# CyberAgentAILab/layout-dm

Measured on NVIDIA H100. Metric: layouts_per_sec_T100_batch1024_N25, higher is better.
Workload: dtype fp16

## Files before the change

layoutdm_b200/csrc/common.cuh:

```cuda
#pragma once
#include <cuda.h>
#include <cuda_bf16.h>
#include <cuda_fp16.h>
#include <cuda_runtime.h>
#include <stdint.h>

namespace ldm {

#define LDM_DEVINL __device__ __forceinline__

constexpr float kLogEps = -69.07755278982137f;

LDM_DEVINL uint32_t smem_u32(const void* p) { return static_cast<uint32_t>(__cvta_generic_to_shared(p)); }
LDM_DEVINL void st_shared_u32(uint32_t addr, uint32_t v) { asm volatile("st.shared.u32 [%0], %1;" ::"r"(addr), "r"(v) : "memory"); }

LDM_DEVINL void pdl_wait() { asm volatile("griddepcontrol.wait;" ::: "memory"); }
LDM_DEVINL void pdl_launch_dependents() { asm volatile("griddepcontrol.launch_dependents;" ::: "memory"); }
LDM_DEVINL void pdl_sync() { pdl_wait(); pdl_launch_dependents(); }

LDM_DEVINL void mbar_init(uint64_t* bar, uint32_t count) {
  asm volatile("mbarrier.init.shared::cta.b64 [%0], %1;" ::"r"(smem_u32(bar)), "r"(count) : "memory");
}
LDM_DEVINL void fence_mbar_init() { asm volatile("fence.mbarrier_init.release.cluster;" ::: "memory"); }

LDM_DEVINL void mbar_arrive_expect_tx(uint64_t* bar, uint32_t bytes) {
  asm volatile("mbarrier.arrive.expect_tx.shared::cta.b64 _, [%0], %1;" ::"r"(smem_u32(bar)), "r"(bytes) : "memory");
}
LDM_DEVINL void mbar_arrive(uint64_t* bar) {
  asm volatile("mbarrier.arrive.shared::cta.b64 _, [%0];" ::"r"(smem_u32(bar)) : "memory");
}
LDM_DEVINL bool mbar_try_wait(uint64_t* bar, uint32_t parity) {
  uint32_t ok;
  asm volatile(
      "{\n\t.reg .pred p;\n\t"
      "mbarrier.try_wait.parity.shared::cta.b64 p, [%1], %2;\n\t"
      "selp.u32 %0, 1, 0, p;\n\t}\n"
      : "=r"(ok)
      : "r"(smem_u32(bar)), "r"(parity)
      : "memory");
  return ok != 0;
}
LDM_DEVINL void mbar_wait(uint64_t* bar, uint32_t parity) {
  uint32_t spins = 0;
  while (!mbar_try_wait(bar, parity)) {
    if (++spins > (1u << 28)) { asm volatile("trap;"); }
  }
}

LDM_DEVINL void tma_prefetch_desc(const CUtensorMap* m) {
  asm volatile("prefetch.tensormap [%0];" ::"l"(reinterpret_cast<uint64_t>(m)) : "memory");
}
LDM_DEVINL void tma_load_2d(void* smem_dst, const CUtensorMap* map, uint64_t* bar, int32_t c0, int32_t c1) {
  asm volatile(
      "cp.async.bulk.tensor.2d.shared::cluster.global.mbarrier::complete_tx::bytes [%0], [%1, {%3, %4}], [%2];"
      ::"r"(smem_u32(smem_dst)), "l"(reinterpret_cast<uint64_t>(map)), "r"(smem_u32(bar)), "r"(c0), "r"(c1)
      : "memory");
}
LDM_DEVINL void tma_store_2d(const CUtensorMap* map, const void* smem_src, int32_t c0, int32_t c1) {
  asm volatile("cp.async.bulk.tensor.2d.global.shared::cta.bulk_group [%0, {%2, %3}], [%1];"
               ::"l"(reinterpret_cast<uint64_t>(map)), "r"(smem_u32(smem_src)), "r"(c0), "r"(c1)
               : "memory");
}
LDM_DEVINL void bulk_copy_g2s(void* smem_dst, const void* src, uint32_t bytes, uint64_t* bar) {
  asm volatile("cp.async.bulk.shared::cluster.global.mbarrier::complete_tx::bytes [%0], [%1], %2, [%3];"
               ::"r"(smem_u32(smem_dst)), "l"(reinterpret_cast<uint64_t>(src)), "r"(bytes), "r"(smem_u32(bar))
               : "memory");
}
LDM_DEVINL void bulk_copy_s2g(void* dst, const void* smem_src, uint32_t bytes) {
  asm volatile("cp.async.bulk.global.shared::cta.bulk_group [%0], [%1], %2;"
               ::"l"(reinterpret_cast<uint64_t>(dst)), "r"(smem_u32(smem_src)), "r"(bytes)
               : "memory");
}
LDM_DEVINL void bulk_commit_group() { asm volatile("cp.async.bulk.commit_group;" ::: "memory"); }
template <int N>
LDM_DEVINL void bulk_wait_group_read() { asm volatile("cp.async.bulk.wait_group.read %0;" ::"n"(N) : "memory"); }
LDM_DEVINL void bulk_wait_group_all() { asm volatile("cp.async.bulk.wait_group 0;" ::: "memory"); }
LDM_DEVINL void fence_proxy_async_smem() { asm volatile("fence.proxy.async.shared::cta;" ::: "memory"); }

template <int R>
LDM_DEVINL void setmaxnreg_inc() { asm volatile("setmaxnreg.inc.sync.aligned.u32 %0;" ::"n"(R)); }
template <int R>
LDM_DEVINL void setmaxnreg_dec() { asm volatile("setmaxnreg.dec.sync.aligned.u32 %0;" ::"n"(R)); }

LDM_DEVINL void named_bar_sync(int id, int nthreads) { asm volatile("bar.sync %0, %1;" ::"r"(id), "r"(nthreads) : "memory"); }

LDM_DEVINL void wgmma_fence() { asm volatile("wgmma.fence.sync.aligned;" ::: "memory"); }
LDM_DEVINL void wgmma_commit() { asm volatile("wgmma.commit_group.sync.aligned;" ::: "memory"); }
template <int N>
LDM_DEVINL void wgmma_wait() { asm volatile("wgmma.wait_group.sync.aligned %0;" ::"n"(N) : "memory"); }
template <int N>
LDM_DEVINL void fence_acc(float (&d)[N]) {
#pragma unroll
  for (int i = 0; i < N; ++i) asm volatile("" : "+f"(d[i])::"memory");
}

template <int SW>
LDM_DEVINL uint64_t make_smem_desc(uint32_t smem_addr) {
  static_assert(SW == 128 || SW == 64, "the kernels use the 128- and 64-byte swizzles");
  uint64_t d = 0;
  d |= static_cast<uint64_t>((smem_addr & 0x3FFFF) >> 4);
  d |= static_cast<uint64_t>(1) << 16;
  d |= static_cast<uint64_t>(8 * SW >> 4) << 32;
  d |= static_cast<uint64_t>(SW == 128 ? 1 : 2) << 62;
  return d;
}

#define LDM_F(i) "+f"(d[i])
#define LDM_ACC128 "{%0, %1, %2, %3, %4, %5, %6, %7, %8, %9, %10, %11, %12, %13, %14, %15, %16, %17, %18, %19, %20, %21, %22, %23, %24, %25, %26, %27, %28, %29, %30, %31, %32, %33, %34, %35, %36, %37, %38, %39, %40, %41, %42, %43, %44, %45, %46, %47, %48, %49, %50, %51, %52, %53, %54, %55, %56, %57, %58, %59, %60, %61, %62, %63, %64, %65, %66, %67, %68, %69, %70, %71, %72, %73, %74, %75, %76, %77, %78, %79, %80, %81, %82, %83, %84, %85, %86, %87, %88, %89, %90, %91, %92, %93, %94, %95, %96, %97, %98, %99, %100, %101, %102, %103, %104, %105, %106, %107, %108, %109, %110, %111, %112, %113, %114, %115, %116, %117, %118, %119, %120, %121, %122, %123, %124, %125, %126, %127}"
#define LDM_OUT128 LDM_F(0), LDM_F(1), LDM_F(2), LDM_F(3), LDM_F(4), LDM_F(5), LDM_F(6), LDM_F(7), LDM_F(8), LDM_F(9), LDM_F(10), LDM_F(11), LDM_F(12), LDM_F(13), LDM_F(14), LDM_F(15), LDM_F(16), LDM_F(17), LDM_F(18), LDM_F(19), LDM_F(20), LDM_F(21), LDM_F(22), LDM_F(23), LDM_F(24), LDM_F(25), LDM_F(26), LDM_F(27), LDM_F(28), LDM_F(29), LDM_F(30), LDM_F(31), LDM_F(32), LDM_F(33), LDM_F(34), LDM_F(35), LDM_F(36), LDM_F(37), LDM_F(38), LDM_F(39), LDM_F(40), LDM_F(41), LDM_F(42), LDM_F(43), LDM_F(44), LDM_F(45), LDM_F(46), LDM_F(47), LDM_F(48), LDM_F(49), LDM_F(50), LDM_F(51), LDM_F(52), LDM_F(53), LDM_F(54), LDM_F(55), LDM_F(56), LDM_F(57), LDM_F(58), LDM_F(59), LDM_F(60), LDM_F(61), LDM_F(62), LDM_F(63), LDM_F(64), LDM_F(65), LDM_F(66), LDM_F(67), LDM_F(68), LDM_F(69), LDM_F(70), LDM_F(71), LDM_F(72), LDM_F(73), LDM_F(74), LDM_F(75), LDM_F(76), LDM_F(77), LDM_F(78), LDM_F(79), LDM_F(80), LDM_F(81), LDM_F(82), LDM_F(83), LDM_F(84), LDM_F(85), LDM_F(86), LDM_F(87), LDM_F(88), LDM_F(89), LDM_F(90), LDM_F(91), LDM_F(92), LDM_F(93), LDM_F(94), LDM_F(95), LDM_F(96), LDM_F(97), LDM_F(98), LDM_F(99), LDM_F(100), LDM_F(101), LDM_F(102), LDM_F(103), LDM_F(104), LDM_F(105), LDM_F(106), LDM_F(107), LDM_F(108), LDM_F(109), LDM_F(110), LDM_F(111), LDM_F(112), LDM_F(113), LDM_F(114), LDM_F(115), LDM_F(116), LDM_F(117), LDM_F(118), LDM_F(119), LDM_F(120), LDM_F(121), LDM_F(122), LDM_F(123), LDM_F(124), LDM_F(125), LDM_F(126), LDM_F(127)
#define LDM_ACC116 "{%0, %1, %2, %3, %4, %5, %6, %7, %8, %9, %10, %11, %12, %13, %14, %15, %16, %17, %18, %19, %20, %21, %22, %23, %24, %25, %26, %27, %28, %29, %30, %31, %32, %33, %34, %35, %36, %37, %38, %39, %40, %41, %42, %43, %44, %45, %46, %47, %48, %49, %50, %51, %52, %53, %54, %55, %56, %57, %58, %59, %60, %61, %62, %63, %64, %65, %66, %67, %68, %69, %70, %71, %72, %73, %74, %75, %76, %77, %78, %79, %80, %81, %82, %83, %84, %85, %86, %87, %88, %89, %90, %91, %92, %93, %94, %95, %96, %97, %98, %99, %100, %101, %102, %103, %104, %105, %106, %107, %108, %109, %110, %111, %112, %113, %114, %115}"
#define LDM_OUT116 LDM_F(0), LDM_F(1), LDM_F(2), LDM_F(3), LDM_F(4), LDM_F(5), LDM_F(6), LDM_F(7), LDM_F(8), LDM_F(9), LDM_F(10), LDM_F(11), LDM_F(12), LDM_F(13), LDM_F(14), LDM_F(15), LDM_F(16), LDM_F(17), LDM_F(18), LDM_F(19), LDM_F(20), LDM_F(21), LDM_F(22), LDM_F(23), LDM_F(24), LDM_F(25), LDM_F(26), LDM_F(27), LDM_F(28), LDM_F(29), LDM_F(30), LDM_F(31), LDM_F(32), LDM_F(33), LDM_F(34), LDM_F(35), LDM_F(36), LDM_F(37), LDM_F(38), LDM_F(39), LDM_F(40), LDM_F(41), LDM_F(42), LDM_F(43), LDM_F(44), LDM_F(45), LDM_F(46), LDM_F(47), LDM_F(48), LDM_F(49), LDM_F(50), LDM_F(51), LDM_F(52), LDM_F(53), LDM_F(54), LDM_F(55), LDM_F(56), LDM_F(57), LDM_F(58), LDM_F(59), LDM_F(60), LDM_F(61), LDM_F(62), LDM_F(63), LDM_F(64), LDM_F(65), LDM_F(66), LDM_F(67), LDM_F(68), LDM_F(69), LDM_F(70), LDM_F(71), LDM_F(72), LDM_F(73), LDM_F(74), LDM_F(75), LDM_F(76), LDM_F(77), LDM_F(78), LDM_F(79), LDM_F(80), LDM_F(81), LDM_F(82), LDM_F(83), LDM_F(84), LDM_F(85), LDM_F(86), LDM_F(87), LDM_F(88), LDM_F(89), LDM_F(90), LDM_F(91), LDM_F(92), LDM_F(93), LDM_F(94), LDM_F(95), LDM_F(96), LDM_F(97), LDM_F(98), LDM_F(99), LDM_F(100), LDM_F(101), LDM_F(102), LDM_F(103), LDM_F(104), LDM_F(105), LDM_F(106), LDM_F(107), LDM_F(108), LDM_F(109), LDM_F(110), LDM_F(111), LDM_F(112), LDM_F(113), LDM_F(114), LDM_F(115)
#define LDM_ACC80 "{%0, %1, %2, %3, %4, %5, %6, %7, %8, %9, %10, %11, %12, %13, %14, %15, %16, %17, %18, %19, %20, %21, %22, %23, %24, %25, %26, %27, %28, %29, %30, %31, %32, %33, %34, %35, %36, %37, %38, %39, %40, %41, %42, %43, %44, %45, %46, %47, %48, %49, %50, %51, %52, %53, %54, %55, %56, %57, %58, %59, %60, %61, %62, %63, %64, %65, %66, %67, %68, %69, %70, %71, %72, %73, %74, %75, %76, %77, %78, %79}"
#define LDM_OUT80 LDM_F(0), LDM_F(1), LDM_F(2), LDM_F(3), LDM_F(4), LDM_F(5), LDM_F(6), LDM_F(7), LDM_F(8), LDM_F(9), LDM_F(10), LDM_F(11), LDM_F(12), LDM_F(13), LDM_F(14), LDM_F(15), LDM_F(16), LDM_F(17), LDM_F(18), LDM_F(19), LDM_F(20), LDM_F(21), LDM_F(22), LDM_F(23), LDM_F(24), LDM_F(25), LDM_F(26), LDM_F(27), LDM_F(28), LDM_F(29), LDM_F(30), LDM_F(31), LDM_F(32), LDM_F(33), LDM_F(34), LDM_F(35), LDM_F(36), LDM_F(37), LDM_F(38), LDM_F(39), LDM_F(40), LDM_F(41), LDM_F(42), LDM_F(43), LDM_F(44), LDM_F(45), LDM_F(46), LDM_F(47), LDM_F(48), LDM_F(49), LDM_F(50), LDM_F(51), LDM_F(52), LDM_F(53), LDM_F(54), LDM_F(55), LDM_F(56), LDM_F(57), LDM_F(58), LDM_F(59), LDM_F(60), LDM_F(61), LDM_F(62), LDM_F(63), LDM_F(64), LDM_F(65), LDM_F(66), LDM_F(67), LDM_F(68), LDM_F(69), LDM_F(70), LDM_F(71), LDM_F(72), LDM_F(73), LDM_F(74), LDM_F(75), LDM_F(76), LDM_F(77), LDM_F(78), LDM_F(79)
#define LDM_ACC64 "{%0, %1, %2, %3, %4, %5, %6, %7, %8, %9, %10, %11, %12, %13, %14, %15, %16, %17, %18, %19, %20, %21, %22, %23, %24, %25, %26, %27, %28, %29, %30, %31, %32, %33, %34, %35, %36, %37, %38, %39, %40, %41, %42, %43, %44, %45, %46, %47, %48, %49, %50, %51, %52, %53, %54, %55, %56, %57, %58, %59, %60, %61, %62, %63}"
#define LDM_OUT64 LDM_F(0), LDM_F(1), LDM_F(2), LDM_F(3), LDM_F(4), LDM_F(5), LDM_F(6), LDM_F(7), LDM_F(8), LDM_F(9), LDM_F(10), LDM_F(11), LDM_F(12), LDM_F(13), LDM_F(14), LDM_F(15), LDM_F(16), LDM_F(17), LDM_F(18), LDM_F(19), LDM_F(20), LDM_F(21), LDM_F(22), LDM_F(23), LDM_F(24), LDM_F(25), LDM_F(26), LDM_F(27), LDM_F(28), LDM_F(29), LDM_F(30), LDM_F(31), LDM_F(32), LDM_F(33), LDM_F(34), LDM_F(35), LDM_F(36), LDM_F(37), LDM_F(38), LDM_F(39), LDM_F(40), LDM_F(41), LDM_F(42), LDM_F(43), LDM_F(44), LDM_F(45), LDM_F(46), LDM_F(47), LDM_F(48), LDM_F(49), LDM_F(50), LDM_F(51), LDM_F(52), LDM_F(53), LDM_F(54), LDM_F(55), LDM_F(56), LDM_F(57), LDM_F(58), LDM_F(59), LDM_F(60), LDM_F(61), LDM_F(62), LDM_F(63)
#define LDM_ACC32 "{%0, %1, %2, %3, %4, %5, %6, %7, %8, %9, %10, %11, %12, %13, %14, %15, %16, %17, %18, %19, %20, %21, %22, %23, %24, %25, %26, %27, %28, %29, %30, %31}"
#define LDM_OUT32 LDM_F(0), LDM_F(1), LDM_F(2), LDM_F(3), LDM_F(4), LDM_F(5), LDM_F(6), LDM_F(7), LDM_F(8), LDM_F(9), LDM_F(10), LDM_F(11), LDM_F(12), LDM_F(13), LDM_F(14), LDM_F(15), LDM_F(16), LDM_F(17), LDM_F(18), LDM_F(19), LDM_F(20), LDM_F(21), LDM_F(22), LDM_F(23), LDM_F(24), LDM_F(25), LDM_F(26), LDM_F(27), LDM_F(28), LDM_F(29), LDM_F(30), LDM_F(31)
template <bool BF16>
LDM_DEVINL void wgmma_ss_n256(float (&d)[128], uint64_t da, uint64_t db, uint32_t accumulate) {
  if constexpr (BF16)
    asm volatile("{\n\t.reg .pred p;\n\tsetp.ne.b32 p, %130, 0;\n\t"
                 "wgmma.mma_async.sync.aligned.m64n256k16.f32.bf16.bf16 " LDM_ACC128 ", %128, %129, p, 1, 1, 0, 0;\n\t}\n"
                 : LDM_OUT128 : "l"(da), "l"(db), "r"(accumulate));
  else
    asm volatile("{\n\t.reg .pred p;\n\tsetp.ne.b32 p, %130, 0;\n\t"
                 "wgmma.mma_async.sync.aligned.m64n256k16.f32.f16.f16 " LDM_ACC128 ", %128, %129, p, 1, 1, 0, 0;\n\t}\n"
                 : LDM_OUT128 : "l"(da), "l"(db), "r"(accumulate));
}
template <bool BF16>
LDM_DEVINL void wgmma_ss_n232(float (&d)[116], uint64_t da, uint64_t db, uint32_t accumulate) {
  if constexpr (BF16)
    asm volatile("{\n\t.reg .pred p;\n\tsetp.ne.b32 p, %118, 0;\n\t"
                 "wgmma.mma_async.sync.aligned.m64n232k16.f32.bf16.bf16 " LDM_ACC116 ", %116, %117, p, 1, 1, 0, 0;\n\t}\n"
                 : LDM_OUT116 : "l"(da), "l"(db), "r"(accumulate));
  else
    asm volatile("{\n\t.reg .pred p;\n\tsetp.ne.b32 p, %118, 0;\n\t"
                 "wgmma.mma_async.sync.aligned.m64n232k16.f32.f16.f16 " LDM_ACC116 ", %116, %117, p, 1, 1, 0, 0;\n\t}\n"
                 : LDM_OUT116 : "l"(da), "l"(db), "r"(accumulate));
}
template <bool BF16>
LDM_DEVINL void wgmma_ss_n160(float (&d)[80], uint64_t da, uint64_t db, uint32_t accumulate) {
  if constexpr (BF16)
    asm volatile("{\n\t.reg .pred p;\n\tsetp.ne.b32 p, %82, 0;\n\t"
                 "wgmma.mma_async.sync.aligned.m64n160k16.f32.bf16.bf16 " LDM_ACC80 ", %80, %81, p, 1, 1, 0, 0;\n\t}\n"
                 : LDM_OUT80 : "l"(da), "l"(db), "r"(accumulate));
  else
    asm volatile("{\n\t.reg .pred p;\n\tsetp.ne.b32 p, %82, 0;\n\t"
                 "wgmma.mma_async.sync.aligned.m64n160k16.f32.f16.f16 " LDM_ACC80 ", %80, %81, p, 1, 1, 0, 0;\n\t}\n"
                 : LDM_OUT80 : "l"(da), "l"(db), "r"(accumulate));
}
template <bool BF16>
LDM_DEVINL void wgmma_ss_n128(float (&d)[64], uint64_t da, uint64_t db, uint32_t accumulate) {
  if constexpr (BF16)
    asm volatile("{\n\t.reg .pred p;\n\tsetp.ne.b32 p, %66, 0;\n\t"
                 "wgmma.mma_async.sync.aligned.m64n128k16.f32.bf16.bf16 " LDM_ACC64 ", %64, %65, p, 1, 1, 0, 0;\n\t}\n"
                 : LDM_OUT64 : "l"(da), "l"(db), "r"(accumulate));
  else
    asm volatile("{\n\t.reg .pred p;\n\tsetp.ne.b32 p, %66, 0;\n\t"
                 "wgmma.mma_async.sync.aligned.m64n128k16.f32.f16.f16 " LDM_ACC64 ", %64, %65, p, 1, 1, 0, 0;\n\t}\n"
                 : LDM_OUT64 : "l"(da), "l"(db), "r"(accumulate));
}
template <bool BF16>
LDM_DEVINL void wgmma_rs_n64_tb(float (&d)[32], const uint32_t (&a)[4], uint64_t db, uint32_t accumulate) {
  if constexpr (BF16)
    asm volatile("{\n\t.reg .pred p;\n\tsetp.ne.b32 p, %37, 0;\n\t"
                 "wgmma.mma_async.sync.aligned.m64n64k16.f32.bf16.bf16 " LDM_ACC32 ", {%32, %33, %34, %35}, %36, p, 1, 1, 1;\n\t}\n"
                 : LDM_OUT32 : "r"(a[0]), "r"(a[1]), "r"(a[2]), "r"(a[3]), "l"(db), "r"(accumulate));
  else
    asm volatile("{\n\t.reg .pred p;\n\tsetp.ne.b32 p, %37, 0;\n\t"
                 "wgmma.mma_async.sync.aligned.m64n64k16.f32.f16.f16 " LDM_ACC32 ", {%32, %33, %34, %35}, %36, p, 1, 1, 1;\n\t}\n"
                 : LDM_OUT32 : "r"(a[0]), "r"(a[1]), "r"(a[2]), "r"(a[3]), "l"(db), "r"(accumulate));
}
#undef LDM_ACC128
#undef LDM_OUT128
#undef LDM_ACC116
#undef LDM_OUT116
#undef LDM_ACC80
#undef LDM_OUT80
#undef LDM_ACC64
#undef LDM_OUT64
#undef LDM_ACC32
#undef LDM_OUT32
#undef LDM_F

enum : int { OP_F16 = 0, OP_BF16 = 1, OP_BF16X3 = 2 };
template <int MODE> struct OpT;
template <> struct OpT<OP_F16> {
  using T = __half; using T2 = __half2;
  static LDM_DEVINL uint32_t pack(float a, float b) { __half2 h = __floats2half2_rn(a, b); return *reinterpret_cast<uint32_t*>(&h); }
  static LDM_DEVINL T from(float a) { return __float2half_rn(a); }
};
template <> struct OpT<OP_BF16> {
  using T = __nv_bfloat16; using T2 = __nv_bfloat162;
  static LDM_DEVINL uint32_t pack(float a, float b) { __nv_bfloat162 h = __floats2bfloat162_rn(a, b); return *reinterpret_cast<uint32_t*>(&h); }
  static LDM_DEVINL T from(float a) { return __float2bfloat16_rn(a); }
};
template <> struct OpT<OP_BF16X3> : OpT<OP_BF16> {
  static LDM_DEVINL void pack_pair(float a, float b, uint32_t& hi, uint32_t& lo) {
    const __nv_bfloat162 h = __floats2bfloat162_rn(a, b);
    const float2 hf = __bfloat1622float2(h);
    const __nv_bfloat162 l = __floats2bfloat162_rn(a - hf.x, b - hf.y);
    hi = *reinterpret_cast<const uint32_t*>(&h); lo = *reinterpret_cast<const uint32_t*>(&l);
  }
  static LDM_DEVINL void from_pair(float a, T& hi, T& lo) { hi = __float2bfloat16_rn(a); lo = __float2bfloat16_rn(a - __bfloat162float(hi)); }
};
template <int MODE> constexpr bool kOpBf16 = MODE != OP_F16;
template <int MODE> constexpr bool kOpSplit = MODE == OP_BF16X3;

template <int MODE> struct OpMaps { CUtensorMap hi; };
template <> struct OpMaps<OP_BF16X3> { CUtensorMap hi, lo; };

LDM_DEVINL uint4 philox4x32_10(uint4 c, uint2 k) {
  constexpr uint32_t M0 = 0xD2511F53u, M1 = 0xCD9E8D57u, W0 = 0x9E3779B9u, W1 = 0xBB67AE85u;
#pragma unroll
  for (int i = 0; i < 10; ++i) {
    const uint32_t hi0 = __umulhi(M0, c.x), lo0 = M0 * c.x;
    const uint32_t hi1 = __umulhi(M1, c.z), lo1 = M1 * c.z;
    c = make_uint4(hi1 ^ c.y ^ k.x, lo1, hi0 ^ c.w ^ k.y, lo0);
    k.x += W0; k.y += W1;
  }
  return c;
}

LDM_DEVINL float u01_from_bits(uint32_t w) { return (static_cast<float>(w >> 9) + 0.5f) * 1.1920928955078125e-07f; }

LDM_DEVINL float gumbel_of(float u) { return -logf(-logf(u + 1e-30f) + 1e-30f); }

LDM_DEVINL uint32_t noise_ctr(uint32_t step, uint32_t stream) { return (step & 0xFFFFFFu) | (stream << 24); }

struct TokenNoise {
  uint2 key; uint32_t tok_lo, tok_hi;
  LDM_DEVINL TokenNoise(unsigned long long seed, unsigned long long b_global0, int b, int S, int s) {
    const unsigned long long tok = (b_global0 + b) * static_cast<unsigned long long>(S) + s;
    key = make_uint2(static_cast<uint32_t>(seed), static_cast<uint32_t>(seed >> 32));
    tok_lo = static_cast<uint32_t>(tok); tok_hi = static_cast<uint32_t>(tok >> 32);
  }
  LDM_DEVINL uint4 block(int blk, uint32_t ctr) const { return philox4x32_10(make_uint4(static_cast<uint32_t>(blk), ctr, tok_lo, tok_hi), key); }
  static LDM_DEVINL int block_of(int c) { return c >> 2; }
  static LDM_DEVINL uint32_t word_of(const uint4& r, int c) { const int k = c & 3; return k == 0 ? r.x : k == 1 ? r.y : k == 2 ? r.z : r.w; }
  LDM_DEVINL void lane_words(int lane, uint32_t ctr, uint32_t (&w)[5]) const {
    const uint4 a = block(block_of(4 * lane), ctr), b = block(block_of(128 + lane), ctr);
    w[0] = word_of(a, 4 * lane); w[1] = word_of(a, 4 * lane + 1); w[2] = word_of(a, 4 * lane + 2); w[3] = word_of(a, 4 * lane + 3);
    w[4] = word_of(b, 128 + lane);
  }
  static constexpr float kGroupMargin = 40.0f;
};

template <int N, class Words>
struct ContractDraw {
  Words words;
  LDM_DEVINL void add_gumbel(const bool (&)[N], float (&lg)[N]) const {
    uint32_t w[N];
    words(1u, w);
#pragma unroll
    for (int j = 0; j < N; ++j) lg[j] += gumbel_of(u01_from_bits(w[j]));
  }
  LDM_DEVINL void exponential(const bool (&)[N], float (&e)[N]) const {
    uint32_t w[N];
    words(0u, w);
#pragma unroll
    for (int j = 0; j < N; ++j) e[j] = -logf(u01_from_bits(w[j]));
  }
};
template <int N, class Words>
LDM_DEVINL ContractDraw<N, Words> contract_draw(Words w) { return ContractDraw<N, Words>{w}; }

struct TorchNoise {
  uint2 key; unsigned long long ctr0; uint32_t tthr;
  __host__ __device__ __forceinline__ TorchNoise(unsigned long long seed, unsigned long long offset, uint32_t tthr_) : ctr0(offset >> 2), tthr(tthr_) {
    key = make_uint2(static_cast<uint32_t>(seed), static_cast<uint32_t>(seed >> 32));
  }
  LDM_DEVINL uint32_t word(uint32_t i) const {
    const uint32_t q = i / tthr, sub = i - q * tthr;
    const unsigned long long ctr = ctr0 + (q >> 2);
    return TokenNoise::word_of(philox4x32_10(make_uint4(static_cast<uint32_t>(ctr), static_cast<uint32_t>(ctr >> 32), sub, 0u), key), q & 3);
  }
  static LDM_DEVINL float uniform(uint32_t w) { return __fmaf_rn(__uint2float_rn(w), 0x1p-32f, 0x1p-33f); }
  static LDM_DEVINL float rand(uint32_t w) { const float u = uniform(w); return u == 1.0f ? 0.0f : u; }
  static LDM_DEVINL float exponential(uint32_t w) { const float u = uniform(w); return u >= 1.0f - 0x1p-24f ? 0x1p-24f : -__logf(u); }
  static constexpr float kGroupMargin = 48.0f;
};

template <int N>
struct TorchDraw {
  TorchNoise exp, gum; uint32_t i_exp, exp_cs, i_gum, S; const int (&cls)[N];
  LDM_DEVINL void add_gumbel(const bool (&on)[N], float (&lg)[N]) const {
#pragma unroll
    for (int j = 0; j < N; ++j) if (on[j]) lg[j] += gumbel_of(TorchNoise::rand(gum.word(i_gum + static_cast<uint32_t>(cls[j]) * S)));
  }
  LDM_DEVINL void exponential(const bool (&on)[N], float (&e)[N]) const {
#pragma unroll
    for (int j = 0; j < N; ++j) e[j] = on[j] ? TorchNoise::exponential(exp.word(i_exp + exp_cs * static_cast<uint32_t>(cls[j]))) : 1.0f;
  }
};

LDM_DEVINL float ex2_approx(float x) {
  float y;
  asm("ex2.approx.ftz.f32 %0, %1;" : "=f"(y) : "f"(x));
  return y;
}

LDM_DEVINL float warp_max(float v) {
#pragma unroll
  for (int o = 16; o > 0; o >>= 1) v = fmaxf(v, __shfl_xor_sync(0xffffffffu, v, o));
  return v;
}
LDM_DEVINL float warp_sum(float v) {
#pragma unroll
  for (int o = 16; o > 0; o >>= 1) v += __shfl_xor_sync(0xffffffffu, v, o);
  return v;
}
LDM_DEVINL double warp_sum_d(double v) {
#pragma unroll
  for (int o = 16; o > 0; o >>= 1) v += __shfl_xor_sync(0xffffffffu, v, o);
  return v;
}

}
```

layoutdm_b200/csrc/gemm_tc.cuh:

```cuda
#pragma once
#include "common.cuh"

namespace ldm {

constexpr int kBM = 128;
constexpr int kWgK = 16;
constexpr int kGemmConsumers = 256;
constexpr int kProducerRegs = 40, kConsumerRegs = 232;

constexpr int gemm_kb(bool split) { return split ? 32 : 64; }

enum : int { EPI_QKV = 0, EPI_RELU = 1, EPI_F32 = 2, EPI_LN = 3 };

struct GemmParams {
  int M, N, K;
  int n_tiles;
  const float* bias;
  void* out;
  int ldo;
  float qscale;
  int qcols;
  const float* resid;
  float* y_out;
  const float* ln_scale;
  const float* ln_shift;
  int adaln;
  float* out32;
  const int* t_layout;
  int n_layouts;
  int rev;
  void* out_lo;
};

template <bool BF16, int N>
LDM_DEVINL void wgmma_ss(float (&d)[N / 2], uint64_t da, uint64_t db, uint32_t accumulate) {
  if constexpr (N == 256) wgmma_ss_n256<BF16>(d, da, db, accumulate);
  else if constexpr (N == 232) wgmma_ss_n232<BF16>(d, da, db, accumulate);
  else if constexpr (N == 160) wgmma_ss_n160<BF16>(d, da, db, accumulate);
  else { static_assert(N == 128, "unsupported wgmma width"); wgmma_ss_n128<BF16>(d, da, db, accumulate); }
}

template <int KB, int PLANES, int A_ROWS, int B_ROWS, int WG_N, int STAGES, bool K_TAIL = true>
struct Ring {
  static constexpr int kKB = KB, kStages = STAGES, kWgN = WG_N;
  static constexpr int kRowBytes = 2 * KB;
  static constexpr int kAPlane = A_ROWS * kRowBytes;
  static constexpr int kABytes = PLANES * kAPlane;
  static constexpr int kBBytes = B_ROWS * kRowBytes;
  static constexpr int kStageBytes = kABytes + PLANES * WG_N * kBBytes;
  static constexpr int kBytes = STAGES * kStageBytes;
  static_assert(kAPlane % (8 * kRowBytes) == 0 && kBBytes % (8 * kRowBytes) == 0, "boxes must keep the swizzle atom's alignment");

  uint8_t* stages;
  uint64_t* full;
  uint64_t* empty;

  LDM_DEVINL Ring(uint8_t* smem, uint64_t* bars) : stages(smem), full(bars), empty(bars + STAGES) {}
  static LDM_DEVINL int num_kb(int K) { return K_TAIL ? (K + KB - 1) / KB : K / KB; }

  template <int MODE>
  static LDM_DEVINL void prefetch(const OpMaps<MODE>& a, const OpMaps<MODE>& b) {
    tma_prefetch_desc(&a.hi);
    tma_prefetch_desc(&b.hi);
    if constexpr (kOpSplit<MODE>) { tma_prefetch_desc(&a.lo); tma_prefetch_desc(&b.lo); }
  }
  LDM_DEVINL void init() const {
    for (int i = 0; i < STAGES; ++i) { mbar_init(&full[i], 1); mbar_init(&empty[i], kGemmConsumers); }
  }
  static LDM_DEVINL void advance(int& s, uint32_t& phase) { if (++s == STAGES) { s = 0; phase ^= 1; } }
  LDM_DEVINL void release_prev(int s) const { mbar_arrive(&empty[s == 0 ? STAGES - 1 : s - 1]); }

  template <int MODE>
  LDM_DEVINL void load_tile(int& s, uint32_t& phase, const OpMaps<MODE>& a, const OpMaps<MODE>& b, int num_kb, int m0, int n0) const {
    static_assert(PLANES == (kOpSplit<MODE> ? 2 : 1), "one operand map per plane");
    for (int kb = 0; kb < num_kb; ++kb) {
      mbar_wait(&empty[s], phase ^ 1);
      uint8_t* st = stages + s * kStageBytes;
      mbar_arrive_expect_tx(&full[s], kStageBytes);
      tma_load_2d(st, &a.hi, &full[s], kb * KB, m0);
#pragma unroll
      for (int wn = 0; wn < WG_N; ++wn) tma_load_2d(st + kABytes + wn * kBBytes, &b.hi, &full[s], kb * KB, n0 + wn * B_ROWS);
      if constexpr (PLANES == 2) {
        tma_load_2d(st + kAPlane, &a.lo, &full[s], kb * KB, m0);
#pragma unroll
        for (int wn = 0; wn < WG_N; ++wn)
          tma_load_2d(st + kABytes + (WG_N + wn) * kBBytes, &b.lo, &full[s], kb * KB, n0 + wn * B_ROWS);
      }
      advance(s, phase);
    }
  }

  template <int MODE>
  LDM_DEVINL void mma_tile(int& s, uint32_t& phase, float (&acc)[B_ROWS / 2], int wm, int wn, int num_kb, int K) const {
    static_assert(PLANES == (kOpSplit<MODE> ? 2 : 1), "one operand map per plane");
    for (int kb = 0; kb < num_kb; ++kb) {
      mbar_wait(&full[s], phase);
      const uint32_t st = smem_u32(stages + s * kStageBytes);
      const uint64_t da = make_smem_desc<kRowBytes>(st + wm * 64 * kRowBytes), da_lo = make_smem_desc<kRowBytes>(st + kAPlane + wm * 64 * kRowBytes);
      const uint64_t db = make_smem_desc<kRowBytes>(st + kABytes + wn * kBBytes);
      const uint64_t db_lo = make_smem_desc<kRowBytes>(st + kABytes + (WG_N + wn) * kBBytes);
      wgmma_fence();
      const auto step = [&](int k) {
        if constexpr (PLANES == 2) {
          wgmma_ss<true, B_ROWS>(acc, da_lo + 2 * k, db + 2 * k, (kb | k) != 0);
          wgmma_ss<true, B_ROWS>(acc, da + 2 * k, db_lo + 2 * k, 1);
          wgmma_ss<true, B_ROWS>(acc, da + 2 * k, db + 2 * k, 1);
        } else {
          wgmma_ss<kOpBf16<MODE>, B_ROWS>(acc, da + 2 * k, db + 2 * k, (kb | k) != 0);
        }
      };
      const bool whole = !K_TAIL || kb * KB + KB <= K;
      if (PLANES == 2 || !whole) step(0);
      if (whole) {
#pragma unroll
        for (int k = PLANES == 2 ? 1 : 0; k < KB / kWgK; ++k) step(k);
      }
      wgmma_commit();
      if (kb > 0) { wgmma_wait<1>(); release_prev(s); }
      advance(s, phase);
    }
    wgmma_wait<0>();
    fence_acc(acc);
    release_prev(s);
  }
};

template <int EPI, bool SPLIT>
constexpr bool kStagedStore = (EPI == EPI_QKV || EPI == EPI_RELU) && !SPLIT;
template <int EPI, int MODE>
constexpr int kGemmThreads = kStagedStore<EPI, kOpSplit<MODE>> ? 384 : 288;

template <int BN_WG, int WG_M, int STAGES, bool SPLIT = false, bool STAGED = false>
struct GemmSmem {
  using R = Ring<gemm_kb(SPLIT), SPLIT ? 2 : 1, 64 * WG_M, BN_WG, 3 - WG_M, STAGES>;
  static constexpr int kStoreCb = 64 * WG_M * 128;
  static constexpr int kStoreBytes = STAGED ? (R::kWgN * BN_WG / 64) * kStoreCb : 0;
  static_assert(!STAGED || BN_WG % 64 == 0, "staged stores go out in 64-column boxes");
  static constexpr int kOffStore = R::kBytes;
  static constexpr int kOffBars = kOffStore + kStoreBytes;
  static constexpr int kOffStat = kOffBars + 256;
  static constexpr int kBytes = kOffStat + 2 * 64 * 16 + 1024 ;
  static_assert(2 * STAGES * 8 <= 256, "barrier block overflow");
  static_assert(kBytes <= 232448, "exceeds the 227 KB of shared memory per CTA");
};

template <int EPI, int N>
LDM_DEVINL void bias_act(const float (&acc)[N], int j, const float* bias, int c, float scale, float (&v)[4]) {
  const float2 b = bias != nullptr ? __ldg(reinterpret_cast<const float2*>(bias + c)) : make_float2(0.0f, 0.0f);
  v[0] = acc[4 * j] + b.x; v[1] = acc[4 * j + 1] + b.y; v[2] = acc[4 * j + 2] + b.x; v[3] = acc[4 * j + 3] + b.y;
#pragma unroll
  for (int e = 0; e < 4; ++e) {
    if constexpr (EPI == EPI_QKV) v[e] *= scale;
    if constexpr (EPI == EPI_RELU) v[e] = fmaxf(v[e], 0.0f);
  }
}

struct LnAffine { const float* gam; const float* bet; float gadd; };
LDM_DEVINL LnAffine ln_affine(const float* scale, const float* shift, int adaln, const int* t_layout, int n_layouts, int m0, int N) {
  LnAffine a{scale, shift, adaln ? 1.0f : 0.0f};
  if (t_layout != nullptr) {
    const int layout = m0 / kBM;
    const int tl = layout < n_layouts ? __ldg(t_layout + layout) : 0;
    a.gam = scale + static_cast<size_t>(tl) * 2 * N; a.bet = a.gam + N; a.gadd = 1.0f;
  }
  return a;
}

template <int BN_WG, int WG_M, int STAGES, int EPI, int MODE>
__global__ void __launch_bounds__(kGemmThreads<EPI, MODE>, 1)
gemm_tc_kernel(const __grid_constant__ OpMaps<MODE> map_a ,
               const __grid_constant__ OpMaps<MODE> map_b ,
               const __grid_constant__ CUtensorMap map_out, const GemmParams p) {
  constexpr bool SPLIT = kOpSplit<MODE>, STAGED = kStagedStore<EPI, SPLIT>;
  using SM = GemmSmem<BN_WG, WG_M, STAGES, SPLIT, STAGED>;
  using O = OpT<MODE>;
  constexpr int kBMt = 64 * WG_M, kAcc = BN_WG / 2;
  static_assert(EPI != EPI_LN || (WG_M == 1 && BN_WG == 232), "LN epilogue is laid out for 464 = 2 x 232 columns");
  static_assert(EPI == EPI_LN || WG_M == 2, "plain epilogues use 128-row tiles");

  extern __shared__ __align__(1024) uint8_t smem_raw[];
  uint8_t* smem = reinterpret_cast<uint8_t*>((reinterpret_cast<uintptr_t>(smem_raw) + 1023) & ~uintptr_t(1023));
  typename SM::R ring(smem, reinterpret_cast<uint64_t*>(smem + SM::kOffBars));

  const int warp = __shfl_sync(0xffffffffu, threadIdx.x >> 5, 0), lane = threadIdx.x & 31;
  const int num_kb = SM::R::num_kb(p.K);
  const int n_mblk = p.M / kBMt, n_work = n_mblk * p.n_tiles;
  const auto tile_m0 = [&](int t) { const int mb = t / p.n_tiles; return (p.rev ? n_mblk - 1 - mb : mb) * kBMt; };
  const auto tile_n0 = [&](int t) { return (t % p.n_tiles) * BN_WG * SM::R::kWgN; };

  if (threadIdx.x == kGemmConsumers) {
    ring.prefetch(map_a, map_b);
    if constexpr (STAGED) tma_prefetch_desc(&map_out);
    ring.init();
    fence_mbar_init();
  }
  __syncthreads();
  pdl_sync();

  if (warp >= kGemmConsumers / 32) {
    if constexpr (STAGED) setmaxnreg_dec<kProducerRegs>();
    if (threadIdx.x == kGemmConsumers) {
      int s = 0;
      uint32_t phase = 0;
      for (int t = blockIdx.x; t < n_work; t += gridDim.x) {
        ring.load_tile(s, phase, map_a, map_b, num_kb, tile_m0(t), tile_n0(t));
        if constexpr (!STAGED) break;
      }
    }
    return;
  }

  if constexpr (STAGED) setmaxnreg_inc<kConsumerRegs>();
  const int wg = warp >> 2;
  const int wm = WG_M == 2 ? wg : 0, wn = WG_M == 2 ? 0 : wg;
  float acc[kAcc];
#pragma unroll
  for (int i = 0; i < kAcc; ++i) acc[i] = 0.0f;
  int s = 0;
  uint32_t phase = 0;
  for (int t = blockIdx.x; t < n_work; t += gridDim.x) {
    const int m0 = tile_m0(t), n0 = tile_n0(t);
    ring.template mma_tile<MODE>(s, phase, acc, wm, wn, num_kb, p.K);

    const int rw = (warp & 3) * 16 + (lane >> 2);
    const int row0 = m0 + wm * 64 + rw, row1 = row0 + 8;
    const int col0 = n0 + wn * BN_WG + 2 * (lane & 3);

    if constexpr (STAGED) {
      float scale = 1.0f;
      if constexpr (EPI == EPI_QKV) scale = (n0 < p.qcols) ? p.qscale : 1.0f;
      const bool leader = (threadIdx.x & 127) == 0;
      uint8_t* stage = smem + SM::kOffStore + wm * 64 * 128;
      const uint32_t stage_u32 = smem_u32(stage);
      const auto wg_bar = [&]() { if (wg == 0) named_bar_sync(2, 128); else named_bar_sync(3, 128); };
      if (leader) bulk_wait_group_read<0>();
      wg_bar();
      const int sw = (rw & 7) << 4;
#pragma unroll
      for (int j = 0; j < BN_WG / 8; ++j) {
        const int c = col0 + 8 * j;
        if (c >= p.N) continue;
        float v[4];
        bias_act<EPI>(acc, j, p.bias, c, scale, v);
        const uint32_t blk = stage_u32 + (j >> 3) * SM::kStoreCb + ((((j & 7) << 4) ^ sw) | (4 * (lane & 3)));
        st_shared_u32(blk + rw * 128, O::pack(v[0], v[1]));
        st_shared_u32(blk + (rw + 8) * 128, O::pack(v[2], v[3]));
      }
      fence_proxy_async_smem();
      wg_bar();
      if (leader) {
#pragma unroll
        for (int cb = 0; cb < BN_WG / 64; ++cb)
          if (n0 + cb * 64 < p.N) tma_store_2d(&map_out, stage + cb * SM::kStoreCb, n0 + cb * 64, m0 + wm * 64);
        bulk_commit_group();
      }
    } else if constexpr (EPI != EPI_LN) {
      float scale = 1.0f;
      if constexpr (EPI == EPI_QKV) scale = (n0 < p.qcols) ? p.qscale : 1.0f;
#pragma unroll
      for (int j = 0; j < BN_WG / 8; ++j) {
        const int c = col0 + 8 * j;
        if (c >= p.N) continue;
        float v[4];
        bias_act<EPI>(acc, j, p.bias, c, scale, v);
        if constexpr (EPI == EPI_F32) {
          float* o = static_cast<float*>(p.out);
          *reinterpret_cast<float2*>(o + static_cast<size_t>(row0) * p.ldo + c) = make_float2(v[0], v[1]);
          *reinterpret_cast<float2*>(o + static_cast<size_t>(row1) * p.ldo + c) = make_float2(v[2], v[3]);
        } else {
          uint32_t* o0 = reinterpret_cast<uint32_t*>(static_cast<typename O::T*>(p.out) + static_cast<size_t>(row0) * p.ldo + c);
          uint32_t* o1 = reinterpret_cast<uint32_t*>(static_cast<typename O::T*>(p.out) + static_cast<size_t>(row1) * p.ldo + c);
          if constexpr (SPLIT) {
            uint32_t* l0 = reinterpret_cast<uint32_t*>(static_cast<typename O::T*>(p.out_lo) + static_cast<size_t>(row0) * p.ldo + c);
            uint32_t* l1 = reinterpret_cast<uint32_t*>(static_cast<typename O::T*>(p.out_lo) + static_cast<size_t>(row1) * p.ldo + c);
            O::pack_pair(v[0], v[1], *o0, *l0);
            O::pack_pair(v[2], v[3], *o1, *l1);
          } else {
            *o0 = O::pack(v[0], v[1]);
            *o1 = O::pack(v[2], v[3]);
          }
        }
      }
    } else {
      float* ssum = reinterpret_cast<float*>(smem + SM::kOffStat);
      float* ssq = ssum + 2 * 64;
      const int N = p.N;
      const float* r0p = p.resid + static_cast<size_t>(row0) * N;
      const float* r1p = p.resid + static_cast<size_t>(row1) * N;
      const float piv0 = __ldg(p.bias) + r0p[0], piv1 = __ldg(p.bias) + r1p[0];
      float s0 = 0.0f, s1 = 0.0f;
#pragma unroll
      for (int j = 0; j < BN_WG / 8; ++j) {
        const int c = col0 + 8 * j;
        const float2 b = __ldg(reinterpret_cast<const float2*>(p.bias + c));
        const float2 ra = *reinterpret_cast<const float2*>(r0p + c), rb = *reinterpret_cast<const float2*>(r1p + c);
        acc[4 * j] += b.x + ra.x; acc[4 * j + 1] += b.y + ra.y;
        acc[4 * j + 2] += b.x + rb.x; acc[4 * j + 3] += b.y + rb.y;
        if (p.y_out != nullptr) {
          *reinterpret_cast<float2*>(p.y_out + static_cast<size_t>(row0) * N + c) = make_float2(acc[4 * j], acc[4 * j + 1]);
          *reinterpret_cast<float2*>(p.y_out + static_cast<size_t>(row1) * N + c) = make_float2(acc[4 * j + 2], acc[4 * j + 3]);
        }
        acc[4 * j] -= piv0; acc[4 * j + 1] -= piv0; acc[4 * j + 2] -= piv1; acc[4 * j + 3] -= piv1;
        s0 += acc[4 * j] + acc[4 * j + 1];
        s1 += acc[4 * j + 2] + acc[4 * j + 3];
      }
#pragma unroll
      for (int o = 1; o <= 2; o <<= 1) {
        s0 += __shfl_xor_sync(0xffffffffu, s0, o);
        s1 += __shfl_xor_sync(0xffffffffu, s1, o);
      }
      if ((lane & 3) == 0) { ssum[wn * 64 + rw] = s0; ssum[wn * 64 + rw + 8] = s1; }
      named_bar_sync(1, kGemmConsumers);
      const float inv_n = 1.0f / static_cast<float>(N);
      const float mean0 = (s0 + ssum[(wn ^ 1) * 64 + rw]) * inv_n, mean1 = (s1 + ssum[(wn ^ 1) * 64 + rw + 8]) * inv_n;
      float q0 = 0.0f, q1 = 0.0f;
#pragma unroll
      for (int j = 0; j < BN_WG / 8; ++j) {
        const float d0 = acc[4 * j] - mean0, d1 = acc[4 * j + 1] - mean0, d2 = acc[4 * j + 2] - mean1, d3 = acc[4 * j + 3] - mean1;
        q0 = fmaf(d0, d0, fmaf(d1, d1, q0));
        q1 = fmaf(d2, d2, fmaf(d3, d3, q1));
      }
#pragma unroll
      for (int o = 1; o <= 2; o <<= 1) {
        q0 += __shfl_xor_sync(0xffffffffu, q0, o);
        q1 += __shfl_xor_sync(0xffffffffu, q1, o);
      }
      if ((lane & 3) == 0) { ssq[wn * 64 + rw] = q0; ssq[wn * 64 + rw + 8] = q1; }
      named_bar_sync(1, kGemmConsumers);
      const float rstd0 = 1.0f / sqrtf(fmaxf((q0 + ssq[(wn ^ 1) * 64 + rw]) * inv_n, 0.0f) + 1e-5f);
      const float rstd1 = 1.0f / sqrtf(fmaxf((q1 + ssq[(wn ^ 1) * 64 + rw + 8]) * inv_n, 0.0f) + 1e-5f);
      const LnAffine a = ln_affine(p.ln_scale, p.ln_shift, p.adaln, p.t_layout, p.n_layouts, m0, N);
      typename O::T* out16 = static_cast<typename O::T*>(p.out);
#pragma unroll
      for (int j = 0; j < BN_WG / 8; ++j) {
        const int c = col0 + 8 * j;
        const float2 g = __ldg(reinterpret_cast<const float2*>(a.gam + c)), h = __ldg(reinterpret_cast<const float2*>(a.bet + c));
        const float v0 = (acc[4 * j] - mean0) * rstd0 * (g.x + a.gadd) + h.x, v1 = (acc[4 * j + 1] - mean0) * rstd0 * (g.y + a.gadd) + h.y;
        const float v2 = (acc[4 * j + 2] - mean1) * rstd1 * (g.x + a.gadd) + h.x, v3 = (acc[4 * j + 3] - mean1) * rstd1 * (g.y + a.gadd) + h.y;
        if constexpr (SPLIT) {
          typename O::T* lo16 = static_cast<typename O::T*>(p.out_lo);
          O::pack_pair(v0, v1, *reinterpret_cast<uint32_t*>(out16 + static_cast<size_t>(row0) * N + c), *reinterpret_cast<uint32_t*>(lo16 + static_cast<size_t>(row0) * N + c));
          O::pack_pair(v2, v3, *reinterpret_cast<uint32_t*>(out16 + static_cast<size_t>(row1) * N + c), *reinterpret_cast<uint32_t*>(lo16 + static_cast<size_t>(row1) * N + c));
        } else {
          *reinterpret_cast<uint32_t*>(out16 + static_cast<size_t>(row0) * N + c) = O::pack(v0, v1);
          *reinterpret_cast<uint32_t*>(out16 + static_cast<size_t>(row1) * N + c) = O::pack(v2, v3);
        }
        if (p.out32 != nullptr) {
          *reinterpret_cast<float2*>(p.out32 + static_cast<size_t>(row0) * N + c) = make_float2(v0, v1);
          *reinterpret_cast<float2*>(p.out32 + static_cast<size_t>(row1) * N + c) = make_float2(v2, v3);
        }
      }
    }
    if constexpr (!STAGED) break;
  }
  if constexpr (STAGED) {
    if ((threadIdx.x & 127) == 0) bulk_wait_group_all();
  }
}

constexpr int kLnThreads = 384, kLnEpiThreads = 96;
struct LnSmem {
  static constexpr int kRows = 64, kWgCols = 232, kCols = 2 * kWgCols;
  using R = Ring<32, 1, kRows, kWgCols, 2, 3, false>;
  static constexpr int kLd = kCols + 8;
  static constexpr int kOffBuf = R::kBytes;
  static constexpr int kOffBars = kOffBuf + kRows * kLd * 4;
  static constexpr int kOffStat = kOffBars + 64;
  static constexpr int kBytes = kOffStat + 3 * kRows * 4 + 1024 ;
  static_assert(kLd * 4 % 16 == 0, "bulk copies need 16-byte aligned rows");
  static_assert(kBytes <= 232448, "exceeds the 227 KB of shared memory per CTA");
};

template <int MODE>
__global__ void __launch_bounds__(kLnThreads, 1)
gemm_ln_kernel(const __grid_constant__ OpMaps<MODE> map_a , const __grid_constant__ OpMaps<MODE> map_b ,
               const GemmParams p) {
  static_assert(!kOpSplit<MODE>, "the split mode runs the fragment-epilogue LN GEMM");
  using SM = LnSmem;
  using O = OpT<MODE>;
  constexpr int kRows = SM::kRows, kWgCols = SM::kWgCols, kLd = SM::kLd, kAcc = kWgCols / 2;
  constexpr int kEpi = kGemmConsumers, kProducer = kEpi + kLnEpiThreads;

  extern __shared__ __align__(1024) uint8_t smem_raw[];
  uint8_t* smem = reinterpret_cast<uint8_t*>((reinterpret_cast<uintptr_t>(smem_raw) + 1023) & ~uintptr_t(1023));
  SM::R ring(smem, reinterpret_cast<uint64_t*>(smem + SM::kOffBars));
  uint64_t* res_full = ring.empty + SM::R::kStages;
  uint64_t* buf_full = res_full + 1;
  float* buf = reinterpret_cast<float*>(smem + SM::kOffBuf);
  float* s_piv = reinterpret_cast<float*>(smem + SM::kOffStat);
  float* s_sum = s_piv + kRows;
  float* s_rstd = s_sum + kRows;

  const int warp = __shfl_sync(0xffffffffu, threadIdx.x >> 5, 0), lane = threadIdx.x & 31;
  const int N = p.N;
  const int num_kb = SM::R::num_kb(p.K);
  const int n_work = p.M / kRows;
  const auto tile_m0 = [&](int t) { return (p.rev ? n_work - 1 - t : t) * kRows; };

  if (threadIdx.x == kProducer) {
    ring.prefetch(map_a, map_b);
    ring.init();
    mbar_init(res_full, 1);
    mbar_init(buf_full, kGemmConsumers);
    fence_mbar_init();
  }
  __syncthreads();
  pdl_sync();

  if (threadIdx.x >= kProducer) {
    if (threadIdx.x == kProducer) {
      uint32_t phase = 0;
      int s = 0;
      for (int t = blockIdx.x; t < n_work; t += gridDim.x) ring.load_tile(s, phase, map_a, map_b, num_kb, tile_m0(t), 0);
    }
    return;
  }

  if (threadIdx.x >= kEpi) {
    const int et = threadIdx.x - kEpi;
    const bool copier = et < 32;
    const uint32_t row_bytes = static_cast<uint32_t>(N) * sizeof(float);
    const float inv_n = 1.0f / static_cast<float>(N);
    constexpr int kVec = kWgCols / 2;
    constexpr int kTotal = kRows * kVec;
    constexpr int kPerThread = (kTotal + kLnEpiThreads - 1) / kLnEpiThreads;
    const auto load_resid = [&](int t) {
      if (lane == 0) mbar_arrive_expect_tx(res_full, kRows * row_bytes);
      __syncwarp();
      const float* src = p.resid + static_cast<size_t>(tile_m0(t)) * N;
      for (int r = lane; r < kRows; r += 32) bulk_copy_g2s(buf + r * kLd, src + static_cast<size_t>(r) * N, row_bytes, res_full);
    };
    const auto store_rows = [&](float* dst) {
      for (int r = lane; r < kRows; r += 32) bulk_copy_s2g(dst + static_cast<size_t>(r) * N, buf + r * kLd, row_bytes);
      bulk_commit_group();
    };
    if (copier) load_resid(blockIdx.x);
    uint32_t bphase = 0;
    for (int t = blockIdx.x; t < n_work; t += gridDim.x) {
      const int m0 = tile_m0(t);
      mbar_wait(buf_full, bphase);
      if (copier && p.y_out != nullptr) store_rows(p.y_out + static_cast<size_t>(m0) * N);
      {
        const int h = (lane >> 2) & 1, q = lane & 3;
#pragma unroll 1
        for (int g = et >> 5; g < kRows / 4; g += kLnEpiThreads / 32) {
          const int r = 4 * g + (lane >> 3);
          const float piv = s_piv[r];
          const float* yr = buf + r * kLd + h * kWgCols + 2 * q;
          float s = 0.0f;
#pragma unroll
          for (int j = 0; j < kWgCols / 8; ++j) {
            const float2 y = *reinterpret_cast<const float2*>(yr + 8 * j);
            s += (y.x - piv) + (y.y - piv);
          }
          s += __shfl_xor_sync(0xffffffffu, s, 1);
          s += __shfl_xor_sync(0xffffffffu, s, 2);
          s += __shfl_xor_sync(0xffffffffu, s, 4);
          float v = 0.0f;
#pragma unroll
          for (int j = 0; j < kWgCols / 8; ++j) {
            const float2 y = *reinterpret_cast<const float2*>(yr + 8 * j);
            const float d0 = fmaf(-s, inv_n, y.x - piv), d1 = fmaf(-s, inv_n, y.y - piv);
            v = fmaf(d0, d0, fmaf(d1, d1, v));
          }
          v += __shfl_xor_sync(0xffffffffu, v, 1);
          v += __shfl_xor_sync(0xffffffffu, v, 2);
          v += __shfl_xor_sync(0xffffffffu, v, 4);
          if ((lane & 7) == 0) { s_sum[r] = s; s_rstd[r] = 1.0f / sqrtf(fmaxf(v * inv_n, 0.0f) + 1e-5f); }
        }
      }
      if (copier) bulk_wait_group_read<0>();
      named_bar_sync(1, kLnEpiThreads);
      const LnAffine a = ln_affine(p.ln_scale, p.ln_shift, p.adaln, p.t_layout, p.n_layouts, m0, N);
      typename O::T* out16 = static_cast<typename O::T*>(p.out);
      const bool keep32 = p.out32 != nullptr;
#pragma unroll 6
      for (int k = 0; k < kPerThread; ++k) {
        const int i = k * kLnEpiThreads + et, r = i / kVec, c = (i - r * kVec) * 4;
        if (i >= kTotal) continue;
        float4* bp = reinterpret_cast<float4*>(buf + r * kLd + c);
        const float4 y = *bp;
        const float4 g = __ldg(reinterpret_cast<const float4*>(a.gam + c)), b = __ldg(reinterpret_cast<const float4*>(a.bet + c));
        const float piv = s_piv[r], s = s_sum[r], rstd = s_rstd[r];
        const float4 v = make_float4(fmaf(fmaf(-s, inv_n, y.x - piv) * rstd, g.x + a.gadd, b.x), fmaf(fmaf(-s, inv_n, y.y - piv) * rstd, g.y + a.gadd, b.y),
                                     fmaf(fmaf(-s, inv_n, y.z - piv) * rstd, g.z + a.gadd, b.z), fmaf(fmaf(-s, inv_n, y.w - piv) * rstd, g.w + a.gadd, b.w));
        *reinterpret_cast<uint2*>(out16 + static_cast<size_t>(m0 + r) * N + c) = make_uint2(O::pack(v.x, v.y), O::pack(v.z, v.w));
        if (keep32) *bp = v;
      }
      if (keep32) fence_proxy_async_smem();
      named_bar_sync(1, kLnEpiThreads);
      if (copier) {
        if (keep32) store_rows(p.out32 + static_cast<size_t>(m0) * N);
        bulk_wait_group_read<0>();
        if (t + static_cast<int>(gridDim.x) < n_work) load_resid(t + gridDim.x);
      }
      bphase ^= 1;
    }
    if (copier) bulk_wait_group_all();
    return;
  }

  const int wn = warp >> 2;
  float acc[kAcc];
  int s = 0;
  uint32_t phase = 0, bphase = 0;
  const int rw = (warp & 3) * 16 + (lane >> 2);
  const int cw = wn * kWgCols + 2 * (lane & 3);
  float* bw = buf + rw * kLd + cw;
  for (int t = blockIdx.x; t < n_work; t += gridDim.x) {
    ring.mma_tile<MODE>(s, phase, acc, 0, wn, num_kb, p.K);
    mbar_wait(res_full, bphase);
    if (cw == 0) { const float b0 = __ldg(p.bias); s_piv[rw] = b0 + bw[0]; s_piv[rw + 8] = b0 + bw[8 * kLd]; }
#pragma unroll
    for (int j = 0; j < kAcc / 4; ++j) {
      const float2 b = __ldg(reinterpret_cast<const float2*>(p.bias + cw + 8 * j));
      float2* y0 = reinterpret_cast<float2*>(bw + 8 * j);
      float2* y1 = reinterpret_cast<float2*>(bw + 8 * kLd + 8 * j);
      const float2 r0 = *y0, r1 = *y1;
      *y0 = make_float2(acc[4 * j] + (b.x + r0.x), acc[4 * j + 1] + (b.y + r0.y));
      *y1 = make_float2(acc[4 * j + 2] + (b.x + r1.x), acc[4 * j + 3] + (b.y + r1.y));
    }
    fence_proxy_async_smem();
    mbar_arrive(buf_full);
    bphase ^= 1;
  }
}

}
```

layoutdm_b200/csrc/ldm_b200.cu:

```cuda
#include <cuda.h>
#include <cuda_runtime.h>

#include <algorithm>
#include <cmath>
#include <cstdarg>
#include <cstdio>
#include <cstdlib>
#include <cstring>
#include <type_traits>
#include <vector>

#include "../../include/ldm_b200.h"
#include "attention.cuh"
#include "common.cuh"
#include "embed.cuh"
#include "gemm_tc.cuh"
#include "posterior_sample.cuh"
#include "relation.cuh"

using namespace ldm;

namespace {

thread_local char g_err[512] = "";
int fail(int code, const char* fmt, ...) {
  va_list ap; va_start(ap, fmt); vsnprintf(g_err, sizeof(g_err), fmt, ap); va_end(ap);
  return code;
}
#define CK(call)                                                                                   \
  do {                                                                                             \
    cudaError_t e__ = (call);                                                                      \
    if (e__ != cudaSuccess) return fail(LDM_ERR_CUDA, "%s failed: %s (%s:%d)", #call, cudaGetErrorString(e__), __FILE__, __LINE__); \
  } while (0)

constexpr int kMaxLayers = 16;
constexpr int kHeadPad = 64;
constexpr int kQkvN = 3 * 8 * kHeadPad;
constexpr int kAttN = 8 * kHeadPad;
constexpr int kMaxLayouts = 32767;
constexpr int kLogitLd = 160;
constexpr int kDModel = 464;
constexpr int kPlainBN = 256;
template <int MODE> constexpr int kPlainStages = kOpSplit<MODE> ? 4 : 3;
constexpr int kHeadBN = 160, kHeadStages = 4;
constexpr int kLnBN = 232, kLnStages = 3;
constexpr int kLnKB = LnSmem::R::kKB;
static_assert(LnSmem::kWgCols == kLnBN && kAttN % kLnKB == 0 && 4 * kDModel % kLnKB == 0 && gemm_kb(true) == kLnKB, "LN GEMM shapes");
template <int MODE> constexpr auto kGemmQkv = gemm_tc_kernel<kPlainBN, 2, kPlainStages<MODE>, EPI_QKV, MODE>;
template <int MODE> constexpr auto kGemmFf1 = gemm_tc_kernel<kPlainBN, 2, kPlainStages<MODE>, EPI_RELU, MODE>;
template <int MODE> constexpr auto kGemmHead = gemm_tc_kernel<kHeadBN, 2, kHeadStages, EPI_F32, MODE>;
template <int MODE> constexpr auto kGemmLn = gemm_tc_kernel<kLnBN, 1, kLnStages, EPI_LN, MODE>;
template <int MODE>
constexpr int kPlainSmem = GemmSmem<kPlainBN, 2, kPlainStages<MODE>, kOpSplit<MODE>, kStagedStore<EPI_QKV, kOpSplit<MODE>>>::kBytes;
constexpr int kHeadSmem = GemmSmem<kHeadBN, 2, kHeadStages>::kBytes;
constexpr int kLnSmem = GemmSmem<kLnBN, 1, kLnStages>::kBytes;
static_assert(GemmSmem<kHeadBN, 2, kHeadStages, true>::kBytes == kHeadSmem && GemmSmem<kLnBN, 1, kLnStages, true>::kBytes == kLnSmem &&
              GemmSmem<kPlainBN, 2, 4, true>::R::kStageBytes == GemmSmem<kPlainBN, 2, 4>::R::kStageBytes,
              "split-mode ring stages must keep the one-plane sizes");
static_assert(kStagedStore<EPI_QKV, false> == kStagedStore<EPI_RELU, false> && kStagedStore<EPI_QKV, true> == kStagedStore<EPI_RELU, true>,
              "QKV and FF1 share one shared-memory size");

using EncodeTiledFn = CUresult (*)(CUtensorMap*, CUtensorMapDataType, cuuint32_t, void*, const cuuint64_t*, const cuuint64_t*,
                                   const cuuint32_t*, const cuuint32_t*, CUtensorMapInterleave, CUtensorMapSwizzle,
                                   CUtensorMapL2promotion, CUtensorMapFloatOOBfill);
EncodeTiledFn g_encode = nullptr;

int load_encode() {
  if (g_encode) return LDM_OK;
  void* fn = nullptr;
  cudaDriverEntryPointQueryResult qres;
  CK(cudaGetDriverEntryPoint("cuTensorMapEncodeTiled", &fn, cudaEnableDefault, &qres));
  if (qres != cudaDriverEntryPointSuccess || fn == nullptr) return fail(LDM_ERR_CUDA, "cuTensorMapEncodeTiled not available");
  g_encode = reinterpret_cast<EncodeTiledFn>(fn);
  return LDM_OK;
}

int make_map(CUtensorMap* m, const void* base, uint64_t rows, uint64_t cols, uint32_t box_rows, int kb, bool bf16) {
  const cuuint64_t dims[2] = {cols, rows};
  const cuuint64_t strides[1] = {cols * 2};
  const cuuint32_t box[2] = {static_cast<cuuint32_t>(kb), box_rows};
  const cuuint32_t estr[2] = {1, 1};
  CUresult r = g_encode(m, bf16 ? CU_TENSOR_MAP_DATA_TYPE_BFLOAT16 : CU_TENSOR_MAP_DATA_TYPE_FLOAT16, 2, const_cast<void*>(base), dims,
                        strides, box, estr, CU_TENSOR_MAP_INTERLEAVE_NONE, kb == 32 ? CU_TENSOR_MAP_SWIZZLE_64B : CU_TENSOR_MAP_SWIZZLE_128B,
                        CU_TENSOR_MAP_L2_PROMOTION_L2_256B, CU_TENSOR_MAP_FLOAT_OOB_FILL_NONE);
  if (r != CUDA_SUCCESS) return fail(LDM_ERR_CUDA, "cuTensorMapEncodeTiled failed (%d) rows=%llu cols=%llu box_rows=%u", (int)r,
                                     (unsigned long long)rows, (unsigned long long)cols, box_rows);
  return LDM_OK;
}

__global__ void logits_scatter_kernel(const float* __restrict__ src, float* __restrict__ dst, int n_layouts, int S, int C) {
  const size_t n = static_cast<size_t>(n_layouts) * S * C;
  for (size_t i = blockIdx.x * static_cast<size_t>(blockDim.x) + threadIdx.x; i < n; i += static_cast<size_t>(gridDim.x) * blockDim.x) {
    const int c = static_cast<int>(i % C); const size_t tok = i / C; const int s = static_cast<int>(tok % S); const size_t b = tok / S;
    dst[(b * 128 + s) * kLogitLd + c] = src[i];
  }
}
__global__ void logits_gather_kernel(const float* __restrict__ src, float* __restrict__ dst, int n_layouts, int S, int C) {
  const size_t n = static_cast<size_t>(n_layouts) * S * C;
  for (size_t i = blockIdx.x * static_cast<size_t>(blockDim.x) + threadIdx.x; i < n; i += static_cast<size_t>(gridDim.x) * blockDim.x) {
    const int c = static_cast<int>(i % C); const size_t tok = i / C; const int s = static_cast<int>(tok % S); const size_t b = tok / S;
    dst[i] = src[(b * 128 + s) * kLogitLd + c];
  }
}
__global__ void fill_ids_kernel(long long* dst, long long v, size_t n) {
  for (size_t i = blockIdx.x * static_cast<size_t>(blockDim.x) + threadIdx.x; i < n; i += static_cast<size_t>(gridDim.x) * blockDim.x) dst[i] = v;
}

}

struct LdmHandle {
  LdmModelDesc desc;
  int C = 0, S = 0, L = 0, T = 0, G = 0;
  int mode = OP_F16;
  bool bf16 = false;
  bool split = false;
  int64_t launches = 0;
  int pdl = 1;
  int debug_stop_after = 0;
  bool prof = false;
  struct ProfRec { int cat; cudaEvent_t a, b; };
  std::vector<ProfRec> prof_recs;
  float *cat_emb = nullptr, *pos = nullptr, *adaln = nullptr, *sched = nullptr, *lae = nullptr;
  void *wqkv[kMaxLayers] = {}, *wo[kMaxLayers] = {}, *w1[kMaxLayers] = {}, *w2[kMaxLayers] = {}, *whead = nullptr;
  float *bqkv[kMaxLayers] = {}, *bo[kMaxLayers] = {}, *b1[kMaxLayers] = {}, *b2[kMaxLayers] = {}, *ln2w[kMaxLayers] = {}, *ln2b[kMaxLayers] = {};
  float *hlnw = nullptr, *hlnb = nullptr;
  CUtensorMap m_wqkv[kMaxLayers], m_wo[kMaxLayers], m_w1[kMaxLayers], m_w2[kMaxLayers], m_whead;
  void *wqkv_lo[kMaxLayers] = {}, *wo_lo[kMaxLayers] = {}, *w1_lo[kMaxLayers] = {}, *w2_lo[kMaxLayers] = {}, *whead_lo = nullptr;
  CUtensorMap m_wqkv_lo[kMaxLayers], m_wo_lo[kMaxLayers], m_w1_lo[kMaxLayers], m_w2_lo[kMaxLayers], m_whead_lo;
  int *qmap = nullptr, *amap = nullptr, *hmap = nullptr;
  int cap = 0;
  void *x16 = nullptr, *qkv16 = nullptr, *att16 = nullptr, *z16 = nullptr, *hid16 = nullptr;
  float *x32 = nullptr, *y32 = nullptr, *logits = nullptr;
  float* rel_lp = nullptr;
  long long* ids[2] = {nullptr, nullptr};
  long long* ids_final = nullptr;
  long long *c_seq = nullptr, *c_seq_orig = nullptr; unsigned char* c_mask = nullptr; float* c_tbl = nullptr;
  CUtensorMap m_x16, m_z16, m_qkv16;
  CUtensorMap m_att16, m_hid16;
  CUtensorMap m_qkv16_st, m_hid16_st;
  void *x16_lo = nullptr, *qkv16_lo = nullptr, *att16_lo = nullptr, *z16_lo = nullptr, *hid16_lo = nullptr;
  CUtensorMap m_x16_lo, m_z16_lo, m_qkv16_lo, m_att16_lo, m_hid16_lo;
  std::vector<void*> owned;
  int use_graph = 1;
  int sweep = 1;
  int num_sms = 0;
  int max_threads_sm = 0;
  int gemm_ctas = 0;
  int fuse_embed = 1;
  cudaStream_t cap_stream = nullptr;
  cudaGraphExec_t graph_exec = nullptr;
  uint64_t graph_key = 0;
  unsigned long long* call_block = nullptr;
  uint64_t ws_generation = 0;
  int64_t graph_launches = 0;
  std::vector<void*> staging;
};

namespace {

template <typename T>
int dev_alloc(LdmHandle* h, T** p, size_t n) {
  CK(cudaMalloc(reinterpret_cast<void**>(p), n * sizeof(T)));
  h->owned.push_back(*p);
  return LDM_OK;
}
template <typename T>
int dev_upload(LdmHandle* h, T** p, const T* src, size_t n) {
  int rc = dev_alloc(h, p, n);
  if (rc) return rc;
  CK(cudaMemcpy(*p, src, n * sizeof(T), cudaMemcpyHostToDevice));
  return LDM_OK;
}

template <typename T>
int dev_upload_tmp(LdmHandle* h, T** p, const T* src, size_t n) {
  CK(cudaMalloc(reinterpret_cast<void**>(p), n * sizeof(T)));
  h->staging.push_back(*p);
  CK(cudaMemcpy(*p, src, n * sizeof(T), cudaMemcpyHostToDevice));
  return LDM_OK;
}
void free_staging(LdmHandle* h) {
  for (void* p : h->staging) cudaFree(p);
  h->staging.clear();
}

int alloc16(LdmHandle* h, void** dst, void** dst_lo, int rows, int cols) {
  const size_t bytes = static_cast<size_t>(rows) * cols * 2;
  CK(cudaMalloc(dst, bytes));
  h->owned.push_back(*dst);
  if (h->split) { CK(cudaMalloc(dst_lo, bytes)); h->owned.push_back(*dst_lo); }
  return LDM_OK;
}

int pack16(const LdmHandle* h, void* dst, void* dst_lo, const float* src_dev, const int* row_map_dev, int dst_rows, int dst_cols, int src_cols,
           cudaStream_t st, const int* col_map_dev = nullptr) {
  const int blocks = 512;
  if (h->mode == OP_BF16X3) pack_weight_kernel<OP_BF16X3><<<blocks, 256, 0, st>>>(src_dev, dst, row_map_dev, col_map_dev, dst_rows, dst_cols, src_cols, dst_lo);
  else if (h->mode == OP_BF16) pack_weight_kernel<OP_BF16><<<blocks, 256, 0, st>>>(src_dev, dst, row_map_dev, col_map_dev, dst_rows, dst_cols, src_cols, nullptr);
  else pack_weight_kernel<OP_F16><<<blocks, 256, 0, st>>>(src_dev, dst, row_map_dev, col_map_dev, dst_rows, dst_cols, src_cols, nullptr);
  CK(cudaGetLastError());
  return LDM_OK;
}

struct WeightField { const float* LdmWeights::*member; const char* name; size_t n; };
std::vector<WeightField> weight_fields(const LdmHandle* h) {
  const size_t d = h->desc.d_model, ff = h->desc.d_ff, L = h->L, T = h->T, C = h->C, S = h->S;
  return {{&LdmWeights::cat_emb, "cat_emb", C * d},         {&LdmWeights::pos_table, "pos_table", S * d},
          {&LdmWeights::in_proj_w, "in_proj_w", L * 3 * d * d}, {&LdmWeights::in_proj_b, "in_proj_b", L * 3 * d},
          {&LdmWeights::out_proj_w, "out_proj_w", L * d * d},   {&LdmWeights::out_proj_b, "out_proj_b", L * d},
          {&LdmWeights::linear1_w, "linear1_w", L * ff * d},    {&LdmWeights::linear1_b, "linear1_b", L * ff},
          {&LdmWeights::linear2_w, "linear2_w", L * d * ff},    {&LdmWeights::linear2_b, "linear2_b", L * d},
          {&LdmWeights::norm1_emb, "norm1_emb", L * T * d},     {&LdmWeights::norm1_w, "norm1_w", L * 2 * d * d},
          {&LdmWeights::norm1_b, "norm1_b", L * 2 * d},         {&LdmWeights::norm2_w, "norm2_w", L * d},
          {&LdmWeights::norm2_b, "norm2_b", L * d},             {&LdmWeights::head_ln_w, "head_ln_w", d},
          {&LdmWeights::head_ln_b, "head_ln_b", d},             {&LdmWeights::head_w, "head_w", C * d}};
}

int pack_weights(LdmHandle* h, const LdmWeights& w, cudaStream_t st) {
  const int d = h->desc.d_model, ff = h->desc.d_ff, L = h->L, T = h->T;
  const auto copy = [&](float* dst, const float* src, size_t n) { return cudaMemcpyAsync(dst, src, n * sizeof(float), cudaMemcpyDeviceToDevice, st); };
  CK(copy(h->cat_emb, w.cat_emb, static_cast<size_t>(h->C) * d));
  CK(copy(h->pos, w.pos_table, static_cast<size_t>(h->S) * d));
  CK(copy(h->hlnw, w.head_ln_w, d));
  CK(copy(h->hlnb, w.head_ln_b, d));
  adaln_table_kernel<<<dim3(T, L), 256, d * sizeof(float), st>>>(w.norm1_emb, w.norm1_w, w.norm1_b, h->adaln, T, d);
  CK(cudaGetLastError());
  int rc;
  for (int l = 0; l < L; ++l) {
    const size_t dd = static_cast<size_t>(d) * d;
    if ((rc = pack16(h, h->wqkv[l], h->wqkv_lo[l], w.in_proj_w + l * 3 * dd, h->qmap, kQkvN, d, d, st))) return rc;
    qkv_bias_kernel<<<(kQkvN + 255) / 256, 256, 0, st>>>(w.in_proj_b + static_cast<size_t>(l) * 3 * d, h->qmap, h->bqkv[l], kQkvN,
                                                        2 * 8 * kHeadPad, kHeadPad, d / h->desc.n_heads);
    CK(cudaGetLastError());
    if ((rc = pack16(h, h->wo[l], h->wo_lo[l], w.out_proj_w + l * dd, nullptr, d, kAttN, d, st, h->amap))) return rc;
    CK(copy(h->bo[l], w.out_proj_b + static_cast<size_t>(l) * d, d));
    if ((rc = pack16(h, h->w1[l], h->w1_lo[l], w.linear1_w + l * ff * static_cast<size_t>(d), nullptr, ff, d, d, st))) return rc;
    CK(copy(h->b1[l], w.linear1_b + static_cast<size_t>(l) * ff, ff));
    if ((rc = pack16(h, h->w2[l], h->w2_lo[l], w.linear2_w + l * ff * static_cast<size_t>(d), nullptr, d, ff, ff, st))) return rc;
    CK(copy(h->b2[l], w.linear2_b + static_cast<size_t>(l) * d, d));
    CK(copy(h->ln2w[l], w.norm2_w + static_cast<size_t>(l) * d, d));
    CK(copy(h->ln2b[l], w.norm2_b + static_cast<size_t>(l) * d, d));
  }
  return pack16(h, h->whead, h->whead_lo, w.head_w, h->hmap, kLogitLd, d, d, st);
}

int make_op_maps(const LdmHandle* h, CUtensorMap* m, CUtensorMap* m_lo, const void* base, const void* base_lo, uint64_t rows, uint64_t cols,
                 uint32_t box_rows, int kb) {
  int rc = make_map(m, base, rows, cols, box_rows, kb, h->bf16);
  if (rc || !h->split) return rc;
  return make_map(m_lo, base_lo, rows, cols, box_rows, kb, h->bf16);
}

template <int MODE>
OpMaps<MODE> op_maps(const CUtensorMap& hi, const CUtensorMap& lo) {
  OpMaps<MODE> m;
  m.hi = hi;
  if constexpr (kOpSplit<MODE>) m.lo = lo;
  else (void)lo;
  return m;
}

void build_schedule(const LdmModelDesc& d, int N, float* out ) {
  const int T = d.num_timesteps, TT = T + 1;
  std::vector<double> att(T + 1), ctt(T + 1);
  att[0] = 1.0; ctt[0] = 0.0;
  for (int i = 0; i < T; ++i) {
    att[i + 1] = static_cast<double>(i) / (T - 1) * (d.att_T - d.att_1) + d.att_1;
    ctt[i + 1] = static_cast<double>(i) / (T - 1) * (d.ctt_T - d.ctt_1) + d.ctt_1;
  }
  auto l1m = [](double la) { return std::log(1.0 - std::exp(la) + 1e-40); };
  for (int i = 0; i < TT; ++i) for (int r = 0; r < 8; ++r) out[r * TT + i] = 0.0f;
  for (int i = 0; i < T; ++i) {
    const double at = att[i + 1] / att[i];
    const double ct = 1.0 - (1.0 - ctt[i + 1]) / (1.0 - ctt[i]);
    const double bt = (1.0 - at - ct) / N;
    out[0 * TT + i] = static_cast<float>(std::log(at));
    out[1 * TT + i] = static_cast<float>(std::log(bt));
    out[2 * TT + i] = static_cast<float>(std::log(ct));
    out[6 * TT + i] = static_cast<float>(l1m(std::log(ct)));
  }
  for (int i = 0; i < TT; ++i) {
    const double a = (i < T) ? att[i + 1] : 1.0, c = (i < T) ? ctt[i + 1] : 0.0;
    const double b = (1.0 - a - c) / N;
    out[3 * TT + i] = static_cast<float>(std::log(a));
    out[4 * TT + i] = static_cast<float>(std::log(b));
    out[5 * TT + i] = static_cast<float>(std::log(c));
    out[7 * TT + i] = static_cast<float>(l1m(std::log(c)));
  }
}

enum : int { CAT_EMBED = 0, CAT_QKV, CAT_ATTN, CAT_OUTPROJ, CAT_FF1, CAT_FF2, CAT_HEAD, CAT_EPILOGUE, CAT_MISC, CAT_COUNT };

struct ProfScope {
  LdmHandle* h; cudaStream_t st; cudaEvent_t b = nullptr;
  ProfScope(LdmHandle* h_, int cat, cudaStream_t st_) : h(h_), st(st_) {
    h->launches++;
    if (h->prof) {
      cudaEvent_t a; cudaEventCreate(&a); cudaEventCreate(&b);
      cudaEventRecord(a, st);
      h->prof_recs.push_back({cat, a, b});
    }
  }
  ~ProfScope() { if (b) cudaEventRecord(b, st); }
};

template <typename... KArgs, typename... Args>
cudaError_t launch_step(const LdmHandle* h, void (*kernel)(KArgs...), dim3 grid, int block, int smem, cudaStream_t st, Args&&... args) {
  cudaLaunchConfig_t cfg = {};
  cfg.gridDim = grid; cfg.blockDim = dim3(block); cfg.dynamicSmemBytes = smem; cfg.stream = st;
  cudaLaunchAttribute at[1];
  cfg.attrs = at; cfg.numAttrs = 0;
  if (h->pdl) { at[0].id = cudaLaunchAttributeProgrammaticStreamSerialization; at[0].val.programmaticStreamSerializationAllowed = 1; cfg.numAttrs = 1; }
  return cudaLaunchKernelEx(&cfg, kernel, std::forward<Args>(args)...);
}

template <int MODE>
int set_smem() {
  constexpr auto attr = cudaFuncAttributeMaxDynamicSharedMemorySize;
  CK(cudaFuncSetAttribute(kGemmQkv<MODE>, attr, kPlainSmem<MODE>));
  CK(cudaFuncSetAttribute(kGemmFf1<MODE>, attr, kPlainSmem<MODE>));
  CK(cudaFuncSetAttribute(kGemmHead<MODE>, attr, kHeadSmem));
  if constexpr (kOpSplit<MODE>) CK(cudaFuncSetAttribute(kGemmLn<MODE>, attr, kLnSmem));
  else CK(cudaFuncSetAttribute(gemm_ln_kernel<MODE>, attr, LnSmem::kBytes));
  CK(cudaFuncSetAttribute(attention_kernel<MODE>, attr, kOpSplit<MODE> ? kAttSmemBytesSplit : kAttSmemBytes));
  return LDM_OK;
}

void free_workspace(LdmHandle* h) {
  void** ws[] = {&h->x16, &h->qkv16, &h->att16, &h->z16, &h->hid16, &h->x16_lo, &h->qkv16_lo, &h->att16_lo, &h->z16_lo, &h->hid16_lo,
                 reinterpret_cast<void**>(&h->x32), reinterpret_cast<void**>(&h->y32),
                 reinterpret_cast<void**>(&h->logits), reinterpret_cast<void**>(&h->ids[0]), reinterpret_cast<void**>(&h->ids[1]),
                 reinterpret_cast<void**>(&h->ids_final), reinterpret_cast<void**>(&h->c_seq), reinterpret_cast<void**>(&h->c_seq_orig),
                 reinterpret_cast<void**>(&h->c_mask), reinterpret_cast<void**>(&h->rel_lp)};
  for (void** p : ws) { if (*p) cudaFree(*p); *p = nullptr; }
  h->cap = 0;
}

int ensure_workspace(LdmHandle* h, int n_layouts) {
  if (n_layouts > kMaxLayouts) return fail(LDM_ERR_UNSUPPORTED, "batch of %d layouts exceeds the %d a call supports", n_layouts, kMaxLayouts);
  if (n_layouts <= h->cap) return LDM_OK;
  CK(cudaDeviceSynchronize());
  free_workspace(h);
  const size_t M = static_cast<size_t>(n_layouts) * kBM;
  const int d = h->desc.d_model, ff = h->desc.d_ff;
  if (h->split) {
    void** lo[] = {&h->x16_lo, &h->qkv16_lo, &h->att16_lo, &h->z16_lo, &h->hid16_lo};
    const size_t cols[] = {static_cast<size_t>(d), static_cast<size_t>(kQkvN), static_cast<size_t>(kAttN), static_cast<size_t>(d), static_cast<size_t>(ff)};
    for (int i = 0; i < 5; ++i) {
      const cudaError_t e = cudaMalloc(lo[i], M * cols[i] * 2);
      if (e != cudaSuccess) {
        cudaGetLastError();
        free_workspace(h);
        return fail(LDM_ERR_CUDA, "split-operand workspace for %d layouts does not fit: %s", n_layouts, cudaGetErrorString(e));
      }
      CK(cudaMemset(*lo[i], 0, M * cols[i] * 2));
    }
  }
  CK(cudaMalloc(&h->x16, M * d * 2));
  CK(cudaMalloc(&h->qkv16, M * kQkvN * 2));
  CK(cudaMalloc(&h->att16, M * kAttN * 2));
  CK(cudaMalloc(&h->z16, M * d * 2));
  CK(cudaMalloc(&h->hid16, M * ff * 2));
  CK(cudaMalloc(reinterpret_cast<void**>(&h->x32), M * d * 4));
  CK(cudaMalloc(reinterpret_cast<void**>(&h->y32), M * d * 4));
  CK(cudaMalloc(reinterpret_cast<void**>(&h->logits), M * kLogitLd * 4));
  const size_t nid = static_cast<size_t>(n_layouts) * h->S;
  CK(cudaMalloc(reinterpret_cast<void**>(&h->ids[0]), nid * 8));
  CK(cudaMalloc(reinterpret_cast<void**>(&h->ids[1]), nid * 8));
  CK(cudaMalloc(reinterpret_cast<void**>(&h->ids_final), nid * 8));
  CK(cudaMalloc(reinterpret_cast<void**>(&h->c_seq), nid * 8));
  CK(cudaMalloc(reinterpret_cast<void**>(&h->c_seq_orig), nid * 8));
  CK(cudaMalloc(reinterpret_cast<void**>(&h->c_mask), nid));
  CK(cudaMemset(h->x16, 0, M * d * 2)); CK(cudaMemset(h->qkv16, 0, M * kQkvN * 2)); CK(cudaMemset(h->att16, 0, M * kAttN * 2));
  CK(cudaMemset(h->z16, 0, M * d * 2)); CK(cudaMemset(h->hid16, 0, M * ff * 2)); CK(cudaMemset(h->x32, 0, M * d * 4));
  CK(cudaMemset(h->y32, 0, M * d * 4));
  CK(cudaMemset(h->logits, 0, M * kLogitLd * 4));
  h->cap = n_layouts;
  h->ws_generation++;
  int rc;
  const int kb = gemm_kb(h->split);
  if ((rc = make_op_maps(h, &h->m_x16, &h->m_x16_lo, h->x16, h->x16_lo, M, d, kBM, kb))) return rc;
  if ((rc = make_op_maps(h, &h->m_z16, &h->m_z16_lo, h->z16, h->z16_lo, M, d, kBM, kb))) return rc;
  if ((rc = make_op_maps(h, &h->m_att16, &h->m_att16_lo, h->att16, h->att16_lo, M, kAttN, 64, kLnKB))) return rc;
  if ((rc = make_op_maps(h, &h->m_hid16, &h->m_hid16_lo, h->hid16, h->hid16_lo, M, ff, 64, kLnKB))) return rc;
  if ((rc = make_op_maps(h, &h->m_qkv16, &h->m_qkv16_lo, h->qkv16, h->qkv16_lo, M, kQkvN, kBM, kHeadPad))) return rc;
  if (!h->split && (rc = make_map(&h->m_qkv16_st, h->qkv16, M, kQkvN, 64, 64, h->bf16))) return rc;
  if (!h->split && (rc = make_map(&h->m_hid16_st, h->hid16, M, ff, 64, 64, h->bf16))) return rc;
  return LDM_OK;
}

template <int MODE>
int launch_denoiser(LdmHandle* h, int n, const long long* ids_in, int t_model, cudaStream_t st, const int* t_layout = nullptr, bool skip_embed = false) {
  const auto maps = [](const CUtensorMap& hi, const CUtensorMap& lo) { return op_maps<MODE>(hi, lo); };
  const int d = h->desc.d_model, ff = h->desc.d_ff, L = h->L, T = h->T;
  const int M = n * kBM;
  const auto grid = [&](int tiles, bool persistent) {
    if (!persistent) return dim3(tiles);
    return dim3(std::min({tiles, h->num_sms, h->gemm_ctas > 0 ? h->gemm_ctas : tiles}));
  };
  const CUtensorMap no_store{};
  constexpr bool kStaged = kStagedStore<EPI_QKV, kOpSplit<MODE>>;
  const auto ln_gemm = [&](const OpMaps<MODE>& a, const OpMaps<MODE>& w, const GemmParams& p) {
    if constexpr (kOpSplit<MODE>) return launch_step(h, kGemmLn<MODE>, grid(M / 64, false), kGemmThreads<EPI_LN, MODE>, kLnSmem, st, a, w, no_store, p);
    else return launch_step(h, gemm_ln_kernel<MODE>, grid(M / 64, true), kLnThreads, LnSmem::kBytes, st, a, w, p);
  };
  int done = 0;
  int dir = 0;
  auto next_rev = [&]() { dir ^= 1; return h->sweep ? dir : 0; };
#define LDM_STAGE_DONE() do { if (h->debug_stop_after && ++done >= h->debug_stop_after) { CK(cudaGetLastError()); return LDM_OK; } } while (0)
  if (!skip_embed) {
    const int warps = n * 128, blocks = (warps * 32 + 255) / 256;
    ProfScope ps(h, CAT_EMBED, st);
    CK(launch_step(h, embed_adaln_kernel<MODE>, dim3(blocks), 256, 0, st, ids_in, (const float*)h->cat_emb, (const float*)h->pos,
                   (const float*)h->adaln, t_model, t_layout, h->x32, h->x16, n, n, h->S, d, h->x16_lo));
  }
  if (!skip_embed) LDM_STAGE_DONE();
  for (int l = 0; l < L; ++l) {
    {
      GemmParams p{M, kQkvN, d, kQkvN / kPlainBN, h->bqkv[l], h->qkv16, kQkvN, 1.0f / sqrtf(static_cast<float>(d / h->desc.n_heads)), 8 * kHeadPad};
      p.rev = next_rev(); p.out_lo = h->qkv16_lo;
      ProfScope ps(h, CAT_QKV, st);
      CK(launch_step(h, kGemmQkv<MODE>, grid(p.n_tiles * n, kStaged), kGemmThreads<EPI_QKV, MODE>, kPlainSmem<MODE>, st, maps(h->m_x16, h->m_x16_lo), maps(h->m_wqkv[l], h->m_wqkv_lo[l]),
                     kStaged ? h->m_qkv16_st : no_store, p));
    }
    LDM_STAGE_DONE();
    {
      ProfScope ps(h, CAT_ATTN, st);
      CK(launch_step(h, attention_kernel<MODE>, dim3(n * h->desc.n_heads), kAttThreads, kOpSplit<MODE> ? kAttSmemBytesSplit : kAttSmemBytes, st,
                     maps(h->m_qkv16, h->m_qkv16_lo), h->att16, h->S, h->desc.n_heads, n, next_rev(), h->att16_lo));
    }
    LDM_STAGE_DONE();
    {
      GemmParams p{M, d, kAttN, 1, h->bo[l], h->z16, d, 1.0f, 0, h->x32, h->y32, h->ln2w[l], h->ln2b[l], 0, nullptr};
      p.rev = next_rev(); p.out_lo = h->z16_lo;
      ProfScope ps(h, CAT_OUTPROJ, st);
      CK(ln_gemm(maps(h->m_att16, h->m_att16_lo), maps(h->m_wo[l], h->m_wo_lo[l]), p));
    }
    LDM_STAGE_DONE();
    {
      GemmParams p{M, ff, d, (ff + kPlainBN - 1) / kPlainBN, h->b1[l], h->hid16, ff, 1.0f, 0};
      p.rev = next_rev(); p.out_lo = h->hid16_lo;
      ProfScope ps(h, CAT_FF1, st);
      CK(launch_step(h, kGemmFf1<MODE>, grid(p.n_tiles * n, kStaged), kGemmThreads<EPI_RELU, MODE>, kPlainSmem<MODE>, st, maps(h->m_z16, h->m_z16_lo), maps(h->m_w1[l], h->m_w1_lo[l]),
                     kStaged ? h->m_hid16_st : no_store, p));
    }
    LDM_STAGE_DONE();
    {
      GemmParams p{M, d, ff, 1, h->b2[l], nullptr, d, 1.0f, 0, h->y32, nullptr, nullptr, nullptr, 0, nullptr};
      if (l + 1 < L) {
        const float* tab = h->adaln + (static_cast<size_t>(l + 1) * T + t_model) * 2 * d;
        p.ln_scale = tab; p.ln_shift = tab + d; p.adaln = 1; p.out32 = h->x32; p.out = h->x16; p.out_lo = h->x16_lo;
        if (t_layout) { p.ln_scale = h->adaln + static_cast<size_t>(l + 1) * T * 2 * d; p.t_layout = t_layout; p.n_layouts = n; }
      } else {
        p.ln_scale = h->hlnw; p.ln_shift = h->hlnb; p.adaln = 0; p.out32 = nullptr; p.out = h->z16; p.out_lo = h->z16_lo;
      }
      p.rev = next_rev();
      ProfScope ps(h, CAT_FF2, st);
      CK(ln_gemm(maps(h->m_hid16, h->m_hid16_lo), maps(h->m_w2[l], h->m_w2_lo[l]), p));
    }
    LDM_STAGE_DONE();
  }
  {
    GemmParams p{M, kLogitLd, d, 1, nullptr, h->logits, kLogitLd, 1.0f, 0};
    p.rev = next_rev();
    ProfScope ps(h, CAT_HEAD, st);
    CK(launch_step(h, kGemmHead<MODE>, grid(n, false), kGemmThreads<EPI_F32, MODE>, kHeadSmem, st, maps(h->m_z16, h->m_z16_lo), maps(h->m_whead, h->m_whead_lo), no_store, p));
  }
#undef LDM_STAGE_DONE
  CK(cudaGetLastError());
  return LDM_OK;
}

int run_denoiser(LdmHandle* h, int n, const long long* ids_in, int t_model, cudaStream_t st, const int* t_layout = nullptr, bool skip_embed = false) {
  switch (h->mode) {
    case OP_BF16X3: return launch_denoiser<OP_BF16X3>(h, n, ids_in, t_model, st, t_layout, skip_embed);
    case OP_BF16: return launch_denoiser<OP_BF16>(h, n, ids_in, t_model, st, t_layout, skip_embed);
    default: return launch_denoiser<OP_F16>(h, n, ids_in, t_model, st, t_layout, skip_embed);
  }
}

int validate_common(LdmHandle* h, int B, const LdmSampling* s) {
  if (!h) return fail(LDM_ERR_INVALID, "null handle");
  if (B <= 0) return fail(LDM_ERR_INVALID, "batch size must be positive (got %d)", B);
  if (!s) return fail(LDM_ERR_INVALID, "null sampling config");
  if (s->mode < 0 || s->mode > LDM_SAMPLING_GUMBEL) return fail(LDM_ERR_INVALID, "unknown sampling mode %d (sampling.py:118 raises NotImplementedError)", s->mode);
  if (s->mode != LDM_SAMPLING_DETERMINISTIC && !(s->temperature > 0.0f)) return fail(LDM_ERR_INVALID, "temperature must be > 0");
  if (s->mode == LDM_SAMPLING_TOP_P && !(s->top_p > 0.0f && s->top_p <= 1.0f)) return fail(LDM_ERR_INVALID, "top_p must be in (0, 1] (sampling.py:96)");
  if (s->mode == LDM_SAMPLING_TOP_K && !(s->top_k >= 1 && s->top_k <= h->C)) return fail(LDM_ERR_INVALID, "top_k out of range");
  return LDM_OK;
}

struct TorchPolicy { uint32_t tthr, delta; };
TorchPolicy torch_policy(const LdmHandle* h, int64_t numel) {
  const int64_t grid = std::min<int64_t>(static_cast<int64_t>(h->num_sms) * (h->max_threads_sm / 256), (numel + 255) / 256);
  const int64_t tthr = 256 * grid;
  return {static_cast<uint32_t>(tthr), static_cast<uint32_t>(((numel - 1) / (tthr * 4) + 1) * 4)};
}
int64_t torch_numel(const LdmHandle* h, int64_t total_layouts) { return total_layouts * h->S * h->C; }
bool torch_batch_fits(const LdmHandle* h, int64_t total_layouts) {
  return total_layouts <= ((int64_t(1) << 31) - 1) / (static_cast<int64_t>(h->S) * h->C);
}

int validate_noise(const LdmHandle* h, int B, int64_t b_global0, const LdmNoise* nz) {
  if (!nz) return fail(LDM_ERR_INVALID, "null noise description");
  if (nz->kind != LDM_NOISE_CONTRACT && nz->kind != LDM_NOISE_TORCH) return fail(LDM_ERR_INVALID, "unknown noise kind %d", nz->kind);
  if (nz->kind == LDM_NOISE_TORCH) {
    if (b_global0 < 0 || nz->total_layouts < b_global0 + B)
      return fail(LDM_ERR_INVALID, "total_layouts=%lld must cover layouts [%lld, %lld)", (long long)nz->total_layouts, (long long)b_global0, (long long)(b_global0 + B));
    if (!torch_batch_fits(h, nz->total_layouts))
      return fail(LDM_ERR_UNSUPPORTED, "torch-generator noise needs total_layouts * S * C < 2^31 (torch splits larger draws)");
    if (nz->offset % 4) return fail(LDM_ERR_INVALID, "a torch generator offset is a multiple of 4 (got %llu)", (unsigned long long)nz->offset);
  }
  return LDM_OK;
}

StepParams base_step_params(const LdmHandle* h, int B) {
  StepParams p{};
  p.n_layouts = B; p.S = h->S; p.C = h->C; p.n_attr = h->desc.n_attr;
  p.pad_id = h->C - 2; p.mask_id = h->C - 1;
  p.constrained = h->desc.q_type == 0;
  for (int g = 0; g < h->desc.n_attr && g < kMaxAttr; ++g) {
    p.grp_start[g] = g == 0 ? 0 : h->desc.n_cat + (g - 1) * h->desc.n_bins;
    p.grp_n[g] = g == 0 ? h->desc.n_cat : h->desc.n_bins;
  }
  p.T = h->T; p.sched = h->sched; p.lae = h->lae;
  p.logits = h->logits; p.ld_logits = kLogitLd;
  p.mode = SAMP_DETERMINISTIC; p.temperature = 1.0f;
  return p;
}

int step_impl(LdmHandle* h, int B, const long long* ids_in, int t_model, int t_post, const LdmCond* cond, const LdmSampling* samp,
              const LdmNoise& noise, uint32_t step_ctr, int t_step, int64_t b_global0, long long* ids_out, float* logits_out, float* logprob_out,
              const float* logits_in, const float* logprob_in, cudaStream_t st, const unsigned long long* call = nullptr,
              bool skip_embed = false, int t_next = -1) {
  if (t_model < 0 || t_model >= h->T || t_post < 0 || t_post >= h->T)
    return fail(LDM_ERR_INVALID, "timestep out of range: t_model=%d t_post=%d T=%d (constrained.py:139)", t_model, t_post, h->T);
  int rc = ensure_workspace(h, B);
  if (rc) return rc;
  if (logprob_in == nullptr) {
    if (logits_in != nullptr) {
      ProfScope ps(h, CAT_MISC, st);
      logits_scatter_kernel<<<1024, 256, 0, st>>>(logits_in, h->logits, B, h->S, h->C);
    } else {
      rc = run_denoiser(h, B, ids_in, t_model, st, nullptr, skip_embed);
      if (rc) return rc;
    }
    if (logits_out != nullptr) {
      ProfScope ps(h, CAT_MISC, st);
      logits_gather_kernel<<<1024, 256, 0, st>>>(h->logits, logits_out, B, h->S, h->C);
    }
  }
  StepParams p = base_step_params(h, B);
  p.t_post = t_post; p.logprob_in = logprob_in; p.ids_in = ids_in;
  if (cond && cond->seq) {
    p.cond_seq = reinterpret_cast<const long long*>(cond->seq); p.cond_mask = cond->mask;
    p.cond_seq_orig = reinterpret_cast<const long long*>(cond->seq_orig); p.refine_tbl = cond->refine_table;
    p.cond_flags = (cond->mask ? COND_HAS_MASK : 0) | (cond->pad_disable ? COND_PAD_DISABLE : 0) |
                   ((cond->seq_orig && cond->refine_table) ? COND_REFINE : 0);
  }
  p.mode = samp->mode; p.temperature = samp->temperature; p.top_p = samp->top_p; p.top_k = samp->top_k;
  p.seed = noise.seed; p.step_ctr = step_ctr; p.b_global0 = b_global0; p.call = call;
  const bool torch_noise = noise.kind == LDM_NOISE_TORCH;
  if (torch_noise) {
    const TorchPolicy tp = torch_policy(h, torch_numel(h, noise.total_layouts));
    p.t_offset = noise.offset; p.t_tthr = tp.tthr; p.t_delta = tp.delta; p.t_step = t_step; p.t_total = noise.total_layouts;
  }
  const auto generic = torch_noise ? posterior_sample_kernel<TorchNoise> : posterior_sample_kernel<TokenNoise>;
  const auto group = torch_noise ? posterior_sample_group_kernel<TorchNoise> : posterior_sample_group_kernel<TokenNoise>;
  p.ids_out = ids_out; p.logprob_out = logprob_out;
  if (t_next >= 0) {
    p.emb_cat = h->cat_emb; p.emb_pos = h->pos; p.emb_adaln = h->adaln + static_cast<size_t>(t_next) * 2 * h->desc.d_model;
    p.emb_x32 = h->x32; p.emb_x16 = h->x16; p.emb_d = h->desc.d_model; p.emb_bf16 = h->bf16 ? 1 : 0;
  }
  const int warps = B * h->S, blocks = (warps * 32 + 255) / 256;
  const bool relation = cond && cond->seq && cond->rel_adj && logprob_in == nullptr && cond->rel_num_update > 0 && t_model >= 10;
  if (relation) {
    if (h->desc.n_attr != 5 || h->desc.n_elem + 1 > kRelMaxNodes || h->desc.n_bins > 32)
      return fail(LDM_ERR_UNSUPPORTED, "relation update needs the c-x-y-w-h layout with <= 31 elements and <= 32 bins");
    if (!h->rel_lp) CK(cudaMalloc(reinterpret_cast<void**>(&h->rel_lp), static_cast<size_t>(h->cap) * h->S * h->C * sizeof(float)));
    StepParams p1 = p;
    p1.cond_flags &= ~COND_PAD_DISABLE; p1.logprob_out = h->rel_lp; p1.emb_adaln = nullptr;
    {
      ProfScope ps(h, CAT_EPILOGUE, st);
      CK(launch_step(h, generic, blocks, 256, 0, st, p1));
    }
    RelationParams r{};
    r.n_layouts = B; r.S = h->S; r.C = h->C; r.n_attr = h->desc.n_attr; r.n_elem = h->desc.n_elem; r.n_cat = h->desc.n_cat;
    r.n_bins = h->desc.n_bins; r.pad_id = h->C - 2; r.lp = h->rel_lp; r.cond_seq = p.cond_seq; r.adj = cond->rel_adj; r.centers = cond->rel_centers;
    const int btot = cond->rel_batch_total > 0 ? cond->rel_batch_total : B;
    r.step = cond->rel_lambda / static_cast<float>(btot * 14);
    r.n_update = cond->rel_num_update;
    {
      ProfScope ps(h, CAT_EPILOGUE, st);
      CK(launch_step(h, relation_update_kernel, B, kRelThreads, 0, st, r));
    }
    StepParams p2 = p;
    p2.logprob_in = h->rel_lp;
    p2.logprob_out = logprob_out;
    {
      ProfScope ps(h, CAT_EPILOGUE, st);
      CK(launch_step(h, generic, blocks, 256, 0, st, p2));
    }
    CK(cudaGetLastError());
    return LDM_OK;
  }
  {
    ProfScope ps(h, CAT_EPILOGUE, st);
    if (group_kernel_applies(p)) CK(launch_step(h, group, blocks, 256, 0, st, p));
    else CK(launch_step(h, generic, blocks, 256, 0, st, p));
  }
  CK(cudaGetLastError());
  return LDM_OK;
}

}

extern "C" {

const char* ldm_last_error(void) { return g_err; }
const char* ldm_version(void) { return "ldm_b200 0.2 (sm_90a, wgmma)"; }

int ldm_create(const LdmModelDesc* desc, const LdmWeights* w, LdmHandle** out) {
  if (!desc || !w || !out) return fail(LDM_ERR_INVALID, "null argument");
  const int d = desc->d_model, ff = desc->d_ff, L = desc->n_layers, T = desc->num_timesteps;
  const int C = desc->n_cat + 4 * desc->n_bins + 2, S = desc->n_elem * desc->n_attr;
  if (d != kDModel || desc->n_heads != 8 || ff != 4 * kDModel)
    return fail(LDM_ERR_UNSUPPORTED, "kernels are built for d_model=464, 8 heads, d_ff=1856 (got %d, %d, %d)", d, desc->n_heads, ff);
  if (L < 1 || L > kMaxLayers || T < 2) return fail(LDM_ERR_UNSUPPORTED, "n_layers must be in [1,%d], T >= 2", kMaxLayers);
  if (C < 129 || C > kLogitLd || S > 125 || S < 1 || desc->n_attr > kMaxAttr || desc->n_attr < 1)
    return fail(LDM_ERR_UNSUPPORTED, "vocabulary C=%d must be in [129,160] and S=%d <= 125", C, S);
  if (desc->q_type != 0 && desc->q_type != 1) return fail(LDM_ERR_INVALID, "q_type must be 0 (constrained) or 1 (vanilla)");
  if (desc->q_type == 0 && desc->n_attr != 5) return fail(LDM_ERR_UNSUPPORTED, "constrained q_type needs the c-x-y-w-h layout (5 attributes)");
  if (desc->operand_dtype < OP_F16 || desc->operand_dtype > OP_BF16X3)
    return fail(LDM_ERR_INVALID, "operand_dtype must be 0 (fp16), 1 (bf16) or 2 (bf16x3), got %d", desc->operand_dtype);
  CK(cudaSetDevice(desc->device));
  cudaDeviceProp prop;
  CK(cudaGetDeviceProperties(&prop, desc->device));
  if (prop.major != 9 || prop.minor != 0) return fail(LDM_ERR_UNSUPPORTED, "sm_90a kernels need a Hopper (CC 9.0) device, found CC %d.%d", prop.major, prop.minor);
  int rc = load_encode();
  if (rc) return rc;

  LdmHandle* h = new LdmHandle();
  h->desc = *desc; h->C = C; h->S = S; h->L = L; h->T = T;
  h->mode = desc->operand_dtype; h->bf16 = h->mode != OP_F16; h->split = h->mode == OP_BF16X3;
  h->G = desc->q_type == 0 ? desc->n_attr : 1;
  if (const char* e = getenv("LDM_PDL")) h->pdl = atoi(e);
  if (const char* e = getenv("LDM_GRAPH")) h->use_graph = atoi(e);
  if (const char* e = getenv("LDM_FUSE_EMBED")) h->fuse_embed = atoi(e);
  if (h->split) h->fuse_embed = 0;
  if (const char* e = getenv("LDM_SWEEP")) h->sweep = atoi(e);
  h->num_sms = prop.multiProcessorCount;
  h->max_threads_sm = prop.maxThreadsPerMultiProcessor;
  if (const char* e = getenv("LDM_GEMM_CTAS")) h->gemm_ctas = std::max(1, atoi(e));
#define TRY(x) do { rc = (x); if (rc) { ldm_destroy(h); return rc; } } while (0)

  TRY(dev_alloc(h, &h->cat_emb, static_cast<size_t>(C) * d));
  TRY(dev_alloc(h, &h->pos, static_cast<size_t>(S) * d));
  TRY(dev_alloc(h, &h->hlnw, static_cast<size_t>(d)));
  TRY(dev_alloc(h, &h->hlnb, static_cast<size_t>(d)));
  TRY(dev_alloc(h, &h->adaln, static_cast<size_t>(L) * T * 2 * d));
  for (int l = 0; l < L; ++l) {
    TRY(alloc16(h, &h->wqkv[l], &h->wqkv_lo[l], kQkvN, d));
    TRY(alloc16(h, &h->wo[l], &h->wo_lo[l], d, kAttN));
    TRY(alloc16(h, &h->w1[l], &h->w1_lo[l], ff, d));
    TRY(alloc16(h, &h->w2[l], &h->w2_lo[l], d, ff));
    TRY(dev_alloc(h, &h->bqkv[l], static_cast<size_t>(kQkvN)));
    TRY(dev_alloc(h, &h->bo[l], static_cast<size_t>(d)));
    TRY(dev_alloc(h, &h->b1[l], static_cast<size_t>(ff)));
    TRY(dev_alloc(h, &h->b2[l], static_cast<size_t>(d)));
    TRY(dev_alloc(h, &h->ln2w[l], static_cast<size_t>(d)));
    TRY(dev_alloc(h, &h->ln2b[l], static_cast<size_t>(d)));
    TRY(make_op_maps(h, &h->m_wqkv[l], &h->m_wqkv_lo[l], h->wqkv[l], h->wqkv_lo[l], kQkvN, d, kPlainBN, gemm_kb(h->split)));
    TRY(make_op_maps(h, &h->m_wo[l], &h->m_wo_lo[l], h->wo[l], h->wo_lo[l], d, kAttN, kLnBN, kLnKB));
    TRY(make_op_maps(h, &h->m_w1[l], &h->m_w1_lo[l], h->w1[l], h->w1_lo[l], ff, d, kPlainBN, gemm_kb(h->split)));
    TRY(make_op_maps(h, &h->m_w2[l], &h->m_w2_lo[l], h->w2[l], h->w2_lo[l], d, ff, kLnBN, kLnKB));
  }
  TRY(alloc16(h, &h->whead, &h->whead_lo, kLogitLd, d));
  TRY(make_op_maps(h, &h->m_whead, &h->m_whead_lo, h->whead, h->whead_lo, kLogitLd, d, kHeadBN, gemm_kb(h->split)));

  const int dh = d / desc->n_heads;
  std::vector<int> qmap(kQkvN);
  for (int r = 0; r < kQkvN; ++r) {
    const int which = r / (8 * kHeadPad), hh = (r % (8 * kHeadPad)) / kHeadPad, j = r % kHeadPad;
    qmap[r] = j < dh ? which * d + hh * dh + j : -1;
  }
  TRY(dev_upload(h, &h->qmap, qmap.data(), qmap.size()));
  std::vector<int> amap(kAttN);
  for (int c = 0; c < kAttN; ++c) amap[c] = (c % kHeadPad) < dh ? (c / kHeadPad) * dh + (c % kHeadPad) : -1;
  TRY(dev_upload(h, &h->amap, amap.data(), amap.size()));
  std::vector<int> hmap(kLogitLd);
  for (int r = 0; r < kLogitLd; ++r) hmap[r] = r < C ? r : -1;
  TRY(dev_upload(h, &h->hmap, hmap.data(), hmap.size()));

  LdmWeights staged{};
  for (const WeightField& f : weight_fields(h)) {
    float* p = nullptr;
    TRY(dev_upload_tmp(h, &p, w->*f.member, f.n));
    staged.*f.member = p;
  }
  TRY(pack_weights(h, staged, nullptr));
  {
    std::vector<float> sch(static_cast<size_t>(h->G) * 8 * (T + 1));
    for (int g = 0; g < h->G; ++g) {
      const int N = desc->q_type == 0 ? (g == 0 ? desc->n_cat : desc->n_bins) + 1 : C - 1;
      build_schedule(*desc, N, sch.data() + static_cast<size_t>(g) * 8 * (T + 1));
    }
    TRY(dev_upload(h, &h->sched, sch.data(), sch.size()));
    TRY(dev_alloc(h, &h->lae, static_cast<size_t>(h->G) * (T + 1) * 4));
    TRY(dev_alloc(h, &h->call_block, static_cast<size_t>(6)));
    lae_table_kernel<<<(h->G * (T + 1) + 127) / 128, 128>>>(h->sched, h->lae, h->G, T + 1);
    if (cudaGetLastError() != cudaSuccess) { ldm_destroy(h); return fail(LDM_ERR_CUDA, "lae_table_kernel launch failed"); }
  }
  if (cudaDeviceSynchronize() != cudaSuccess) { ldm_destroy(h); return fail(LDM_ERR_CUDA, "weight packing failed: %s", cudaGetErrorString(cudaGetLastError())); }
  free_staging(h);

  TRY(h->mode == OP_BF16X3 ? set_smem<OP_BF16X3>() : h->mode == OP_BF16 ? set_smem<OP_BF16>() : set_smem<OP_F16>());
#undef TRY
  *out = h;
  return LDM_OK;
}

int ldm_destroy(LdmHandle* h) {
  if (!h) return LDM_OK;
  cudaSetDevice(h->desc.device);
  cudaDeviceSynchronize();
  if (h->graph_exec) cudaGraphExecDestroy(h->graph_exec);
  if (h->cap_stream) cudaStreamDestroy(h->cap_stream);
  for (void* p : h->owned) cudaFree(p);
  free_staging(h);
  free_workspace(h);
  if (h->c_tbl) cudaFree(h->c_tbl);
  delete h;
  return LDM_OK;
}

int ldm_load_weights(LdmHandle* h, const LdmWeights* w, void* stream) {
  if (!h || !w) return fail(LDM_ERR_INVALID, "null argument");
  CK(cudaSetDevice(h->desc.device));
  for (const WeightField& f : weight_fields(h)) {
    const float* p = w->*f.member;
    if (!p) return fail(LDM_ERR_INVALID, "LdmWeights.%s is null", f.name);
    cudaPointerAttributes a{};
    if (cudaPointerGetAttributes(&a, p) != cudaSuccess || (a.type != cudaMemoryTypeDevice && a.type != cudaMemoryTypeManaged) ||
        a.device != h->desc.device) {
      cudaGetLastError();
      return fail(LDM_ERR_INVALID, "LdmWeights.%s is not device memory of device %d", f.name, h->desc.device);
    }
  }
  return pack_weights(h, *w, static_cast<cudaStream_t>(stream));
}

int ldm_step_noise(LdmHandle* h, int32_t B, const int64_t* ids_in, int32_t t_model, int32_t t_post, const LdmCond* cond,
                   const LdmSampling* sampling, const LdmNoise* noise, uint32_t step_ctr, int64_t b_global0, int64_t* ids_out,
                   float* logits_out, float* logprob_out, const float* logits_in, const float* logprob_in, void* stream) {
  int rc = validate_common(h, B, sampling);
  if (rc) return rc;
  if ((rc = validate_noise(h, B, b_global0, noise))) return rc;
  if (!ids_in || !ids_out) return fail(LDM_ERR_INVALID, "ids_in / ids_out must not be null");
  CK(cudaSetDevice(h->desc.device));
  return step_impl(h, B, reinterpret_cast<const long long*>(ids_in), t_model, t_post, cond, sampling, *noise, step_ctr, 0, b_global0,
                   reinterpret_cast<long long*>(ids_out), logits_out, logprob_out, logits_in, logprob_in, static_cast<cudaStream_t>(stream));
}

int ldm_step(LdmHandle* h, int32_t B, const int64_t* ids_in, int32_t t_model, int32_t t_post, const LdmCond* cond,
             const LdmSampling* sampling, uint64_t seed, uint32_t step_ctr, int64_t b_global0, int64_t* ids_out,
             float* logits_out, float* logprob_out, const float* logits_in, const float* logprob_in, void* stream) {
  const LdmNoise noise{LDM_NOISE_CONTRACT, seed, 0, 0};
  return ldm_step_noise(h, B, ids_in, t_model, t_post, cond, sampling, &noise, step_ctr, b_global0, ids_out, logits_out, logprob_out,
                        logits_in, logprob_in, stream);
}

int64_t ldm_noise_advance(const LdmHandle* h, int64_t total_layouts, const LdmSampling* sampling, int32_t n_steps) {
  if (!h || !sampling || total_layouts <= 0 || n_steps < 0) return fail(LDM_ERR_INVALID, "bad ldm_noise_advance arguments");
  if (!torch_batch_fits(h, total_layouts))
    return fail(LDM_ERR_UNSUPPORTED, "torch-generator noise needs total_layouts * S * C < 2^31 (torch splits larger draws)");
  if (sampling->mode == LDM_SAMPLING_DETERMINISTIC) return 0;
  const int64_t per_step = static_cast<int64_t>(torch_policy(h, torch_numel(h, total_layouts)).delta) * (sampling->mode == LDM_SAMPLING_GUMBEL ? 2 : 1);
  return per_step * n_steps;
}

int ldm_debug_torch_noise(const LdmHandle* h, int64_t numel, uint64_t seed, uint64_t offset, int32_t which, float* out, void* stream) {
  if (!h || !out || numel <= 0 || numel >= (int64_t(1) << 31) || offset % 4 || (which != 0 && which != 1))
    return fail(LDM_ERR_INVALID, "bad ldm_debug_torch_noise arguments");
  CK(cudaSetDevice(h->desc.device));
  const TorchPolicy tp = torch_policy(h, numel);
  torch_noise_tap_kernel<<<1024, 256, 0, static_cast<cudaStream_t>(stream)>>>(TorchNoise(seed, offset, tp.tthr), static_cast<uint32_t>(numel), which, out);
  CK(cudaGetLastError());
  return LDM_OK;
}

namespace {

int run_loop(LdmHandle* h, int B, int n_steps, const int32_t* t_model, const int32_t* t_post, const LdmCond* cond, const LdmSampling* sampling,
             const LdmNoise& noise, int64_t b_global0, const long long* ids_init, long long* ids_out, long long* ids_trace, cudaStream_t st,
             const unsigned long long* call) {
  const size_t nid = static_cast<size_t>(B) * h->S;
  const long long* cur = nullptr;
  if (ids_init) cur = ids_init;
  else if (cond && cond->seq) cur = reinterpret_cast<const long long*>(cond->seq);
  else {
    ProfScope ps(h, CAT_MISC, st);
    fill_ids_kernel<<<256, 256, 0, st>>>(h->ids[0], static_cast<long long>(h->C - 1), nid);
    cur = h->ids[0];
  }
  for (int i = 0; i < n_steps; ++i) {
    long long* dst;
    if (ids_trace) dst = ids_trace + static_cast<size_t>(i) * nid;
    else if (i == n_steps - 1) dst = ids_out;
    else dst = (cur == h->ids[0]) ? h->ids[1] : h->ids[0];
    const bool fuse = h->fuse_embed != 0;
    int rc = step_impl(h, B, cur, t_model[i], t_post[i], cond, sampling, noise, static_cast<uint32_t>(i), i, b_global0, dst, nullptr, nullptr, nullptr, nullptr, st, call,
                       fuse && i > 0, (fuse && i + 1 < n_steps) ? t_model[i + 1] : -1);
    if (rc) return rc;
    cur = dst;
  }
  if (ids_trace) CK(cudaMemcpyAsync(ids_out, cur, nid * 8, cudaMemcpyDeviceToDevice, st));
  return LDM_OK;
}

uint64_t fnv1a(uint64_t hsh, const void* data, size_t n) {
  const unsigned char* b = static_cast<const unsigned char*>(data);
  for (size_t i = 0; i < n; ++i) { hsh ^= b[i]; hsh *= 1099511628211ull; }
  return hsh;
}

}

int ldm_sample_loop_noise(LdmHandle* h, int32_t B, int32_t n_steps, const int32_t* t_model, const int32_t* t_post, const LdmCond* cond,
                          const LdmSampling* sampling, const LdmNoise* noise, int64_t b_global0, const int64_t* ids_init, int64_t* ids_out,
                          int64_t* ids_trace, void* stream) {
  int rc = validate_common(h, B, sampling);
  if (rc) return rc;
  if ((rc = validate_noise(h, B, b_global0, noise))) return rc;
  if (n_steps < 1 || !t_model || !t_post || !ids_out) return fail(LDM_ERR_INVALID, "bad loop arguments");
  for (int i = 0; i < n_steps; ++i) {
    if (t_model[i] < 0 || t_model[i] >= h->T || t_post[i] < 0 || t_post[i] >= h->T)
      return fail(LDM_ERR_INVALID, "timestep out of range: t_model=%d t_post=%d T=%d (constrained.py:139)", t_model[i], t_post[i], h->T);
    if (i > 0 && t_model[i] >= t_model[i - 1]) return fail(LDM_ERR_INVALID, "timesteps must be strictly decreasing (base.py:361-362 raises NotImplementedError)");
  }
  CK(cudaSetDevice(h->desc.device));
  cudaStream_t st = static_cast<cudaStream_t>(stream);
  rc = ensure_workspace(h, B);
  if (rc) return rc;
  const size_t nid = static_cast<size_t>(B) * h->S;
  const bool has_cond = cond && cond->seq;
  if (!h->use_graph || h->prof || ids_trace || h->debug_stop_after || (has_cond && cond->rel_adj))
    return run_loop(h, B, n_steps, t_model, t_post, has_cond ? cond : nullptr, sampling, *noise, b_global0, reinterpret_cast<const long long*>(ids_init),
                    reinterpret_cast<long long*>(ids_out), reinterpret_cast<long long*>(ids_trace), st, nullptr);

  LdmCond gc{};
  if (has_cond) {
    if (reinterpret_cast<const long long*>(cond->seq) != h->c_seq) CK(cudaMemcpyAsync(h->c_seq, cond->seq, nid * 8, cudaMemcpyDeviceToDevice, st));
    gc.seq = reinterpret_cast<const int64_t*>(h->c_seq);
    if (cond->mask) {
      if (cond->mask != h->c_mask) CK(cudaMemcpyAsync(h->c_mask, cond->mask, nid, cudaMemcpyDeviceToDevice, st));
      gc.mask = h->c_mask;
    }
    if (cond->seq_orig && cond->refine_table) {
      if (reinterpret_cast<const long long*>(cond->seq_orig) != h->c_seq_orig) CK(cudaMemcpyAsync(h->c_seq_orig, cond->seq_orig, nid * 8, cudaMemcpyDeviceToDevice, st));
      const size_t tb = static_cast<size_t>(h->C) * h->C * 4;
      if (!h->c_tbl) CK(cudaMalloc(reinterpret_cast<void**>(&h->c_tbl), tb));
      if (cond->refine_table != h->c_tbl) CK(cudaMemcpyAsync(h->c_tbl, cond->refine_table, tb, cudaMemcpyDeviceToDevice, st));
      gc.seq_orig = reinterpret_cast<const int64_t*>(h->c_seq_orig); gc.refine_table = h->c_tbl;
    }
    gc.pad_disable = cond->pad_disable;
  }
  if (ids_init && reinterpret_cast<const long long*>(ids_init) != h->ids[1]) CK(cudaMemcpyAsync(h->ids[1], ids_init, nid * 8, cudaMemcpyDeviceToDevice, st));
  const TorchPolicy tp = noise->kind == LDM_NOISE_TORCH ? torch_policy(h, torch_numel(h, noise->total_layouts)) : TorchPolicy{0, 0};
  const unsigned long long blk[6] = {noise->seed, static_cast<unsigned long long>(b_global0), noise->offset, tp.tthr, tp.delta,
                                     static_cast<unsigned long long>(noise->total_layouts)};
  CK(cudaMemcpyAsync(h->call_block, blk, sizeof(blk), cudaMemcpyHostToDevice, st));

  uint64_t key = 1469598103934665603ull;
  const int32_t head[7] = {B, n_steps, has_cond ? 1 + (gc.mask ? 2 : 0) + (gc.seq_orig ? 4 : 0) + (gc.pad_disable ? 8 : 0) : 0, ids_init ? 1 : 0, h->pdl, h->fuse_embed,
                           noise->kind};
  key = fnv1a(key, head, sizeof(head));
  key = fnv1a(key, t_model, sizeof(int32_t) * n_steps);
  key = fnv1a(key, t_post, sizeof(int32_t) * n_steps);
  key = fnv1a(key, sampling, sizeof(LdmSampling));
  key = fnv1a(key, &h->ws_generation, sizeof(h->ws_generation));
  if (!h->graph_exec || key != h->graph_key) {
    if (h->graph_exec) { CK(cudaStreamSynchronize(st)); cudaGraphExecDestroy(h->graph_exec); h->graph_exec = nullptr; }
    if (!h->cap_stream) CK(cudaStreamCreateWithFlags(&h->cap_stream, cudaStreamNonBlocking));
    const int64_t l0 = h->launches;
    bool ok = cudaStreamBeginCapture(h->cap_stream, cudaStreamCaptureModeThreadLocal) == cudaSuccess;
    cudaGraph_t g = nullptr;
    if (ok) {
      const LdmNoise staged{noise->kind, 0, 0, noise->total_layouts};
      rc = run_loop(h, B, n_steps, t_model, t_post, has_cond ? &gc : nullptr, sampling, staged, 0, ids_init ? h->ids[1] : nullptr, h->ids_final, nullptr,
                    h->cap_stream, h->call_block);
      ok = cudaStreamEndCapture(h->cap_stream, &g) == cudaSuccess && g != nullptr && rc == LDM_OK;
      h->graph_launches = h->launches - l0;
      h->launches = l0;
    }
    if (ok) ok = cudaGraphInstantiate(&h->graph_exec, g, 0) == cudaSuccess;
    if (g) cudaGraphDestroy(g);
    if (!ok) {
      cudaGetLastError();
      h->graph_exec = nullptr; h->use_graph = 0;
      return run_loop(h, B, n_steps, t_model, t_post, has_cond ? &gc : nullptr, sampling, *noise, b_global0, ids_init ? h->ids[1] : nullptr,
                      reinterpret_cast<long long*>(ids_out), nullptr, st, nullptr);
    }
    h->graph_key = key;
  }
  CK(cudaGraphLaunch(h->graph_exec, st));
  h->launches += h->graph_launches;
  if (reinterpret_cast<long long*>(ids_out) != h->ids_final) CK(cudaMemcpyAsync(ids_out, h->ids_final, nid * 8, cudaMemcpyDeviceToDevice, st));
  return LDM_OK;
}

int ldm_sample_loop(LdmHandle* h, int32_t B, int32_t n_steps, const int32_t* t_model, const int32_t* t_post, const LdmCond* cond,
                    const LdmSampling* sampling, uint64_t seed, int64_t b_global0, const int64_t* ids_init, int64_t* ids_out,
                    int64_t* ids_trace, void* stream) {
  const LdmNoise noise{LDM_NOISE_CONTRACT, seed, 0, 0};
  return ldm_sample_loop_noise(h, B, n_steps, t_model, t_post, cond, sampling, &noise, b_global0, ids_init, ids_out, ids_trace, stream);
}

int ldm_sample_host(LdmHandle* h, int32_t B, int32_t n_steps, const int32_t* t_model, const int32_t* t_post,
                    const int64_t* cond_seq, const uint8_t* cond_mask, const int64_t* cond_seq_orig, const float* refine_table,
                    int32_t pad_disable, const LdmSampling* sampling, uint64_t seed, int64_t b_global0, const int64_t* ids_init,
                    int64_t* ids_out, void* stream, int64_t* h2d_bytes, int64_t* d2h_bytes) {
  int rc = validate_common(h, B, sampling);
  if (rc) return rc;
  if (!ids_out) return fail(LDM_ERR_INVALID, "ids_out_host must not be null");
  CK(cudaSetDevice(h->desc.device));
  cudaStream_t st = static_cast<cudaStream_t>(stream);
  rc = ensure_workspace(h, B);
  if (rc) return rc;
  const size_t nid = static_cast<size_t>(B) * h->S;
  int64_t up = 0;
  LdmCond cond{};
  if (cond_seq) {
    CK(cudaMemcpyAsync(h->c_seq, cond_seq, nid * 8, cudaMemcpyHostToDevice, st)); up += nid * 8;
    cond.seq = reinterpret_cast<const int64_t*>(h->c_seq);
    if (cond_mask) { CK(cudaMemcpyAsync(h->c_mask, cond_mask, nid, cudaMemcpyHostToDevice, st)); up += nid; cond.mask = h->c_mask; }
    if (cond_seq_orig && refine_table) {
      CK(cudaMemcpyAsync(h->c_seq_orig, cond_seq_orig, nid * 8, cudaMemcpyHostToDevice, st)); up += nid * 8;
      cond.seq_orig = reinterpret_cast<const int64_t*>(h->c_seq_orig);
      const size_t tb = static_cast<size_t>(h->C) * h->C * 4;
      if (!h->c_tbl) CK(cudaMalloc(reinterpret_cast<void**>(&h->c_tbl), tb));
      CK(cudaMemcpyAsync(h->c_tbl, refine_table, tb, cudaMemcpyHostToDevice, st)); up += tb;
      cond.refine_table = h->c_tbl;
    }
    cond.pad_disable = pad_disable;
  }
  const int64_t* init_dev = nullptr;
  if (ids_init) {
    CK(cudaMemcpyAsync(h->ids[1], ids_init, nid * 8, cudaMemcpyHostToDevice, st)); up += nid * 8;
    init_dev = reinterpret_cast<const int64_t*>(h->ids[1]);
  }
  rc = ldm_sample_loop(h, B, n_steps, t_model, t_post, cond_seq ? &cond : nullptr, sampling, seed, b_global0, init_dev,
                       reinterpret_cast<int64_t*>(h->ids_final), nullptr, stream);
  if (rc) return rc;
  CK(cudaMemcpyAsync(ids_out, h->ids_final, nid * 8, cudaMemcpyDeviceToHost, st));
  CK(cudaStreamSynchronize(st));
  if (h2d_bytes) *h2d_bytes = up;
  if (d2h_bytes) *d2h_bytes = static_cast<int64_t>(nid * 8);
  return LDM_OK;
}

int ldm_q_sample(LdmHandle* h, int32_t B, const int64_t* x0, const int32_t* t, uint64_t seed, int64_t b_global0, int64_t* xt, void* stream) {
  if (!h || !x0 || !t || !xt || B <= 0) return fail(LDM_ERR_INVALID, "bad ldm_q_sample arguments");
  CK(cudaSetDevice(h->desc.device));
  StepParams p = base_step_params(h, B);
  p.seed = seed; p.b_global0 = b_global0;
  cudaStream_t st = static_cast<cudaStream_t>(stream);
  const int warps = B * h->S, blocks = (warps * 32 + 255) / 256;
  {
    ProfScope ps(h, CAT_MISC, st);
    q_sample_kernel<<<blocks, 256, 0, st>>>(p, reinterpret_cast<const long long*>(x0), t, reinterpret_cast<long long*>(xt));
  }
  CK(cudaGetLastError());
  return LDM_OK;
}

int ldm_decode(LdmHandle* h, int32_t B, const int64_t* ids, const float* centers, float* bbox, int64_t* label, uint8_t* mask, void* stream) {
  if (!h || !ids || !bbox || !label || !mask || B <= 0) return fail(LDM_ERR_INVALID, "bad ldm_decode arguments");
  if (h->desc.n_attr != 5) return fail(LDM_ERR_UNSUPPORTED, "decode needs the c-x-y-w-h token layout");
  CK(cudaSetDevice(h->desc.device));
  cudaStream_t st = static_cast<cudaStream_t>(stream);
  const int n = B * h->desc.n_elem;
  {
    ProfScope ps(h, CAT_MISC, st);
    decode_kernel<<<(n + 255) / 256, 256, 0, st>>>(reinterpret_cast<const long long*>(ids), centers, bbox, reinterpret_cast<long long*>(label), mask,
                                                  B, h->desc.n_elem, h->desc.n_attr, h->desc.n_cat, h->desc.n_bins);
  }
  CK(cudaGetLastError());
  return LDM_OK;
}

int ldm_make_cond(LdmHandle* h, int32_t B, int32_t cond_type, const int64_t* label, const float* bbox, const uint8_t* elem_mask,
                  const float* centers, int64_t* seq, uint8_t* mask, int64_t* seq_orig, void* stream) {
  if (!h || !label || !bbox || !elem_mask || !seq || !mask || B <= 0) return fail(LDM_ERR_INVALID, "bad ldm_make_cond arguments");
  if (h->desc.n_attr != 5) return fail(LDM_ERR_UNSUPPORTED, "make_cond needs the c-x-y-w-h token layout");
  if (cond_type < COND_TYPE_C || cond_type > COND_TYPE_GT)
    return fail(LDM_ERR_UNSUPPORTED, "cond_type %d: only c / cwh / refinement / gt are built on the device (task.py:27-151 raises NotImplementedError for unknown types)", cond_type);
  if (cond_type == COND_TYPE_REFINEMENT && !seq_orig) return fail(LDM_ERR_INVALID, "refinement needs seq_orig_out");
  CK(cudaSetDevice(h->desc.device));
  cudaStream_t st = static_cast<cudaStream_t>(stream);
  const int n = B * h->desc.n_elem;
  const double dd = 1.0 / h->desc.n_bins;
  {
    ProfScope ps(h, CAT_MISC, st);
    make_cond_kernel<<<(n + 255) / 256, 256, 0, st>>>(reinterpret_cast<const long long*>(label), bbox, elem_mask, centers,
                                                     reinterpret_cast<long long*>(seq), mask,
                                                     cond_type == COND_TYPE_REFINEMENT ? reinterpret_cast<long long*>(seq_orig) : nullptr, B,
                                                     h->desc.n_elem, h->desc.n_cat, h->desc.n_bins, h->C - 2, h->C - 1, cond_type,
                                                     static_cast<float>(dd), static_cast<float>(1.0 - dd));
  }
  CK(cudaGetLastError());
  return LDM_OK;
}

namespace {

int run_denoiser_per_layout_t(LdmHandle* h, int B, const long long* ids, const int32_t* t_dev, cudaStream_t st) {
  int rc = ensure_workspace(h, B);
  if (rc) return rc;
  return run_denoiser(h, B, ids, 0, st, t_dev);
}

}

int ldm_predict_start(LdmHandle* h, int32_t B, const int64_t* xt_ids, const int32_t* t_dev, float* log_x0_out, float* logits_out, void* stream) {
  if (!h || !xt_ids || !t_dev || !log_x0_out || B <= 0) return fail(LDM_ERR_INVALID, "bad ldm_predict_start arguments");
  CK(cudaSetDevice(h->desc.device));
  cudaStream_t st = static_cast<cudaStream_t>(stream);
  int rc = run_denoiser_per_layout_t(h, B, reinterpret_cast<const long long*>(xt_ids), t_dev, st);
  if (rc) return rc;
  if (logits_out) { ProfScope ps(h, CAT_MISC, st); logits_gather_kernel<<<1024, 256, 0, st>>>(h->logits, logits_out, B, h->S, h->C); }
  StepParams p = base_step_params(h, B);
  p.ids_in = reinterpret_cast<const long long*>(xt_ids); p.t_layout = t_dev; p.lx0_out = log_x0_out;
  const int blocks = (B * h->S * 32 + 255) / 256;
  { ProfScope ps(h, CAT_EPILOGUE, st); CK(launch_step(h, posterior_sample_kernel<>, blocks, 256, 0, st, p)); }
  CK(cudaGetLastError());
  return LDM_OK;
}

int ldm_q_posterior(LdmHandle* h, int32_t B, const float* log_x_start, const int64_t* xt_ids, const int32_t* t_dev, float* out, void* stream) {
  if (!h || !log_x_start || !xt_ids || !t_dev || !out || B <= 0) return fail(LDM_ERR_INVALID, "bad ldm_q_posterior arguments");
  CK(cudaSetDevice(h->desc.device));
  cudaStream_t st = static_cast<cudaStream_t>(stream);
  StepParams p = base_step_params(h, B);
  p.ids_in = reinterpret_cast<const long long*>(xt_ids); p.t_layout = t_dev; p.lx0_in = log_x_start; p.logprob_out = out;
  const int blocks = (B * h->S * 32 + 255) / 256;
  { ProfScope ps(h, CAT_EPILOGUE, st); CK(launch_step(h, posterior_sample_kernel<>, blocks, 256, 0, st, p)); }
  CK(cudaGetLastError());
  return LDM_OK;
}

namespace {
int q_pred_impl(LdmHandle* h, int32_t B, const float* log_x, const int32_t* t_dev, float* out, void* stream, int one_step) {
  if (!h || !log_x || !t_dev || !out || B <= 0) return fail(LDM_ERR_INVALID, "bad ldm_q_pred arguments");
  CK(cudaSetDevice(h->desc.device));
  cudaStream_t st = static_cast<cudaStream_t>(stream);
  StepParams p = base_step_params(h, B);
  p.t_layout = t_dev;
  { ProfScope ps(h, CAT_MISC, st); q_pred_kernel<<<1024, 256, 0, st>>>(p, log_x, out, one_step); }
  CK(cudaGetLastError());
  return LDM_OK;
}
}

int ldm_q_pred(LdmHandle* h, int32_t B, const float* log_x_start, const int32_t* t_dev, float* out, void* stream) {
  return q_pred_impl(h, B, log_x_start, t_dev, out, stream, 0);
}
int ldm_q_pred_one_timestep(LdmHandle* h, int32_t B, const float* log_x_t, const int32_t* t_dev, float* out, void* stream) {
  return q_pred_impl(h, B, log_x_t, t_dev, out, stream, 1);
}

int ldm_gumbel_argmax(LdmHandle* h, int32_t B, const float* logits, uint64_t seed, int64_t b_global0, int64_t* ids_out, void* stream) {
  if (!h || !logits || !ids_out || B <= 0) return fail(LDM_ERR_INVALID, "bad ldm_gumbel_argmax arguments");
  CK(cudaSetDevice(h->desc.device));
  cudaStream_t st = static_cast<cudaStream_t>(stream);
  const int blocks = (B * h->S * 32 + 255) / 256;
  { ProfScope ps(h, CAT_MISC, st); gumbel_argmax_kernel<<<blocks, 256, 0, st>>>(logits, reinterpret_cast<long long*>(ids_out), B, h->S, h->C, seed, b_global0); }
  CK(cudaGetLastError());
  return LDM_OK;
}

int ldm_vb_terms(LdmHandle* h, int32_t B, const int64_t* x0_ids, const int64_t* xt_ids, const int32_t* t_dev, float mask_weight_mask,
                 float mask_weight_other, float* kl_out, float* nll_out, float* kl_aux_out, float* log_model_prob_out,
                 int64_t* x0_recon_out, int64_t* xtm1_recon_out, void* stream) {
  if (!h || !x0_ids || !xt_ids || !t_dev || !kl_out || !nll_out || B <= 0) return fail(LDM_ERR_INVALID, "bad ldm_vb_terms arguments");
  CK(cudaSetDevice(h->desc.device));
  cudaStream_t st = static_cast<cudaStream_t>(stream);
  int rc = run_denoiser_per_layout_t(h, B, reinterpret_cast<const long long*>(xt_ids), t_dev, st);
  if (rc) return rc;
  float* tok = h->y32;
  const size_t nt = static_cast<size_t>(B) * h->S;
  VbParams v{};
  v.sp = base_step_params(h, B);
  v.sp.ids_in = reinterpret_cast<const long long*>(xt_ids); v.sp.t_layout = t_dev; v.sp.logprob_out = log_model_prob_out;
  v.x0 = reinterpret_cast<const long long*>(x0_ids); v.w_mask = mask_weight_mask; v.w_other = mask_weight_other;
  v.kl_tok = tok; v.nll_tok = tok + nt; v.aux_tok = kl_aux_out ? tok + 2 * nt : nullptr;
  v.x0_recon = reinterpret_cast<long long*>(x0_recon_out); v.xtm1_recon = reinterpret_cast<long long*>(xtm1_recon_out);
  const int blocks = (B * h->S * 32 + 255) / 256, rblocks = (B * 32 + 255) / 256;
  { ProfScope ps(h, CAT_EPILOGUE, st); CK(launch_step(h, vb_terms_kernel, blocks, 256, 0, st, v)); }
  { ProfScope ps(h, CAT_MISC, st); CK(launch_step(h, row_mean_kernel, rblocks, 256, 0, st, (const float*)v.kl_tok, kl_out, B, h->S)); }
  { ProfScope ps(h, CAT_MISC, st); CK(launch_step(h, row_mean_kernel, rblocks, 256, 0, st, (const float*)v.nll_tok, nll_out, B, h->S)); }
  if (kl_aux_out) { ProfScope ps(h, CAT_MISC, st); CK(launch_step(h, row_mean_kernel, rblocks, 256, 0, st, (const float*)v.aux_tok, kl_aux_out, B, h->S)); }
  CK(cudaGetLastError());
  return LDM_OK;
}

int64_t ldm_launch_count(const LdmHandle* h) { return h ? h->launches : 0; }

int ldm_profile_begin(LdmHandle* h) {
  if (!h) return fail(LDM_ERR_INVALID, "null handle");
  h->prof = true;
  return LDM_OK;
}

int ldm_profile_end(LdmHandle* h, float* ms_per_category, int64_t* launches_per_category, int32_t n_categories) {
  if (!h) return fail(LDM_ERR_INVALID, "null handle");
  h->prof = false;
  CK(cudaDeviceSynchronize());
  for (int i = 0; i < n_categories; ++i) { if (ms_per_category) ms_per_category[i] = 0.0f; if (launches_per_category) launches_per_category[i] = 0; }
  for (auto& r : h->prof_recs) {
    float ms = 0.0f;
    cudaEventElapsedTime(&ms, r.a, r.b);
    if (r.cat < n_categories) { if (ms_per_category) ms_per_category[r.cat] += ms; if (launches_per_category) launches_per_category[r.cat]++; }
    cudaEventDestroy(r.a); cudaEventDestroy(r.b);
  }
  h->prof_recs.clear();
  return LDM_OK;
}

int ldm_debug_set_stop_after(LdmHandle* h, int32_t n_launches) {
  if (!h) return fail(LDM_ERR_INVALID, "null handle");
  h->debug_stop_after = n_launches;
  return LDM_OK;
}

int64_t ldm_debug_read(const LdmHandle* h, const char* name, void* dst, int64_t capacity_bytes, int32_t n_layouts) {
  if (!h || !name || n_layouts > h->cap) return -1;
  const size_t M = static_cast<size_t>(n_layouts) * kBM;
  const int d = h->desc.d_model, ff = h->desc.d_ff;
  const void* src = nullptr; size_t bytes = 0;
  if (!strcmp(name, "x32")) { src = h->x32; bytes = M * d * 4; }
  else if (!strcmp(name, "y32")) { src = h->y32; bytes = M * d * 4; }
  else if (!strcmp(name, "x16")) { src = h->x16; bytes = M * d * 2; }
  else if (!strcmp(name, "z16")) { src = h->z16; bytes = M * d * 2; }
  else if (!strcmp(name, "att16")) { src = h->att16; bytes = M * kAttN * 2; }
  else if (!strcmp(name, "qkv16")) { src = h->qkv16; bytes = M * kQkvN * 2; }
  else if (!strcmp(name, "hid16")) { src = h->hid16; bytes = M * ff * 2; }
  else if (!strcmp(name, "logits")) { src = h->logits; bytes = M * kLogitLd * 4; }
  else if (!strcmp(name, "x16_lo")) { src = h->x16_lo; bytes = M * d * 2; }
  else if (!strcmp(name, "z16_lo")) { src = h->z16_lo; bytes = M * d * 2; }
  else if (!strcmp(name, "att16_lo")) { src = h->att16_lo; bytes = M * kAttN * 2; }
  else if (!strcmp(name, "qkv16_lo")) { src = h->qkv16_lo; bytes = M * kQkvN * 2; }
  else if (!strcmp(name, "hid16_lo")) { src = h->hid16_lo; bytes = M * ff * 2; }
  else return -1;
  if (!h->split && strstr(name, "_lo") != nullptr) return -1;
  if (dst && capacity_bytes >= static_cast<int64_t>(bytes)) {
    if (cudaDeviceSynchronize() != cudaSuccess) return -2;
    if (cudaMemcpy(dst, src, bytes, cudaMemcpyDeviceToHost) != cudaSuccess) return -2;
  }
  return static_cast<int64_t>(bytes);
}
int32_t ldm_num_classes(const LdmHandle* h) { return h ? h->C : 0; }
int32_t ldm_seq_len(const LdmHandle* h) { return h ? h->S : 0; }

int64_t ldm_get_schedule(const LdmHandle* h, float* dst, int64_t capacity) {
  if (!h) return 0;
  const int64_t n = static_cast<int64_t>(h->G) * 8 * (h->T + 1);
  if (dst && capacity >= n) cudaMemcpy(dst, h->sched, n * 4, cudaMemcpyDeviceToHost);
  return n;
}
int64_t ldm_get_adaln_table(const LdmHandle* h, float* dst, int64_t capacity) {
  if (!h) return 0;
  const int64_t n = static_cast<int64_t>(h->L) * h->T * 2 * h->desc.d_model;
  if (dst && capacity >= n) cudaMemcpy(dst, h->adaln, n * 4, cudaMemcpyDeviceToHost);
  return n;
}

}
```

Before: 983.5.

## Add row-block GEMM kernel keeping A resident in smem for QKV and FF1

Adds a persistent row-block GEMM for the non-split QKV and FF1 projections. It loads the 128-row A block into shared memory once and streams weight column tiles through a ring, with two consumer warpgroups alternating tiles and staged TMA stores. Work is split into column ranges per row block so the grid fills the SMs at small M. This is meant to cut repeated A reloads and per-tile launch overhead, at the cost of a more complex schedule and higher shared-memory use. The old staged-store path in the generic kernel is removed, so that kernel becomes non-persistent.

```diff
diff --git a/layoutdm_b200/csrc/common.cuh b/layoutdm_b200/csrc/common.cuh
--- a/layoutdm_b200/csrc/common.cuh
+++ b/layoutdm_b200/csrc/common.cuh
@@ -83,6 +83,7 @@
 LDM_DEVINL void setmaxnreg_dec() { asm volatile("setmaxnreg.dec.sync.aligned.u32 %0;" ::"n"(R)); }
 
 LDM_DEVINL void named_bar_sync(int id, int nthreads) { asm volatile("bar.sync %0, %1;" ::"r"(id), "r"(nthreads) : "memory"); }
+LDM_DEVINL void named_bar_arrive(int id, int nthreads) { asm volatile("bar.arrive %0, %1;" ::"r"(id), "r"(nthreads) : "memory"); }
 
 LDM_DEVINL void wgmma_fence() { asm volatile("wgmma.fence.sync.aligned;" ::: "memory"); }
 LDM_DEVINL void wgmma_commit() { asm volatile("wgmma.commit_group.sync.aligned;" ::: "memory"); }
diff --git a/layoutdm_b200/csrc/gemm_tc.cuh b/layoutdm_b200/csrc/gemm_tc.cuh
--- a/layoutdm_b200/csrc/gemm_tc.cuh
+++ b/layoutdm_b200/csrc/gemm_tc.cuh
@@ -30,6 +30,7 @@
   int n_layouts;
   int rev;
   void* out_lo;
+  int n_ranges;
 };
 
 template <bool BF16, int N>
@@ -40,7 +41,9 @@
   else { static_assert(N == 128, "unsupported wgmma width"); wgmma_ss_n128<BF16>(d, da, db, accumulate); }
 }
 
-template <int KB, int PLANES, int A_ROWS, int B_ROWS, int WG_N, int STAGES, bool K_TAIL = true>
+struct NoKbHook { LDM_DEVINL void operator()(int) const {} };
+
+template <int KB, int PLANES, int A_ROWS, int B_ROWS, int WG_N, int STAGES, bool K_TAIL = true, int CONSUMERS = kGemmConsumers>
 struct Ring {
   static constexpr int kKB = KB, kStages = STAGES, kWgN = WG_N;
   static constexpr int kRowBytes = 2 * KB;
@@ -65,23 +68,25 @@
     if constexpr (kOpSplit<MODE>) { tma_prefetch_desc(&a.lo); tma_prefetch_desc(&b.lo); }
   }
   LDM_DEVINL void init() const {
-    for (int i = 0; i < STAGES; ++i) { mbar_init(&full[i], 1); mbar_init(&empty[i], kGemmConsumers); }
+    for (int i = 0; i < STAGES; ++i) { mbar_init(&full[i], 1); mbar_init(&empty[i], CONSUMERS); }
   }
   static LDM_DEVINL void advance(int& s, uint32_t& phase) { if (++s == STAGES) { s = 0; phase ^= 1; } }
   LDM_DEVINL void release_prev(int s) const { mbar_arrive(&empty[s == 0 ? STAGES - 1 : s - 1]); }
 
-  template <int MODE>
-  LDM_DEVINL void load_tile(int& s, uint32_t& phase, const OpMaps<MODE>& a, const OpMaps<MODE>& b, int num_kb, int m0, int n0) const {
+  template <int MODE, class OnKb = NoKbHook>
+  LDM_DEVINL void load_tile(int& s, uint32_t& phase, const OpMaps<MODE>& a, const OpMaps<MODE>& b, int num_kb, int m0, int n0,
+                            OnKb on_kb = {}) const {
     static_assert(PLANES == (kOpSplit<MODE> ? 2 : 1), "one operand map per plane");
     for (int kb = 0; kb < num_kb; ++kb) {
+      on_kb(kb);
       mbar_wait(&empty[s], phase ^ 1);
       uint8_t* st = stages + s * kStageBytes;
       mbar_arrive_expect_tx(&full[s], kStageBytes);
-      tma_load_2d(st, &a.hi, &full[s], kb * KB, m0);
+      if constexpr (A_ROWS > 0) tma_load_2d(st, &a.hi, &full[s], kb * KB, m0);
 #pragma unroll
       for (int wn = 0; wn < WG_N; ++wn) tma_load_2d(st + kABytes + wn * kBBytes, &b.hi, &full[s], kb * KB, n0 + wn * B_ROWS);
+      if constexpr (PLANES == 2 && A_ROWS > 0) tma_load_2d(st + kAPlane, &a.lo, &full[s], kb * KB, m0);
       if constexpr (PLANES == 2) {
-        tma_load_2d(st + kAPlane, &a.lo, &full[s], kb * KB, m0);
 #pragma unroll
         for (int wn = 0; wn < WG_N; ++wn)
           tma_load_2d(st + kABytes + (WG_N + wn) * kBBytes, &b.lo, &full[s], kb * KB, n0 + wn * B_ROWS);
@@ -125,19 +130,12 @@
   }
 };
 
-template <int EPI, bool SPLIT>
-constexpr bool kStagedStore = (EPI == EPI_QKV || EPI == EPI_RELU) && !SPLIT;
-template <int EPI, int MODE>
-constexpr int kGemmThreads = kStagedStore<EPI, kOpSplit<MODE>> ? 384 : 288;
-
-template <int BN_WG, int WG_M, int STAGES, bool SPLIT = false, bool STAGED = false>
+constexpr int kGemmThreads = 288;
+
+template <int BN_WG, int WG_M, int STAGES, bool SPLIT = false>
 struct GemmSmem {
   using R = Ring<gemm_kb(SPLIT), SPLIT ? 2 : 1, 64 * WG_M, BN_WG, 3 - WG_M, STAGES>;
-  static constexpr int kStoreCb = 64 * WG_M * 128;
-  static constexpr int kStoreBytes = STAGED ? (R::kWgN * BN_WG / 64) * kStoreCb : 0;
-  static_assert(!STAGED || BN_WG % 64 == 0, "staged stores go out in 64-column boxes");
-  static constexpr int kOffStore = R::kBytes;
-  static constexpr int kOffBars = kOffStore + kStoreBytes;
+  static constexpr int kOffBars = R::kBytes;
   static constexpr int kOffStat = kOffBars + 256;
   static constexpr int kBytes = kOffStat + 2 * 64 * 16 + 1024 ;
   static_assert(2 * STAGES * 8 <= 256, "barrier block overflow");
@@ -167,12 +165,11 @@
 }
 
 template <int BN_WG, int WG_M, int STAGES, int EPI, int MODE>
-__global__ void __launch_bounds__(kGemmThreads<EPI, MODE>, 1)
+__global__ void __launch_bounds__(kGemmThreads, 1)
 gemm_tc_kernel(const __grid_constant__ OpMaps<MODE> map_a ,
-               const __grid_constant__ OpMaps<MODE> map_b ,
-               const __grid_constant__ CUtensorMap map_out, const GemmParams p) {
-  constexpr bool SPLIT = kOpSplit<MODE>, STAGED = kStagedStore<EPI, SPLIT>;
-  using SM = GemmSmem<BN_WG, WG_M, STAGES, SPLIT, STAGED>;
+               const __grid_constant__ OpMaps<MODE> map_b , const GemmParams p) {
+  constexpr bool SPLIT = kOpSplit<MODE>;
+  using SM = GemmSmem<BN_WG, WG_M, STAGES, SPLIT>;
   using O = OpT<MODE>;
   constexpr int kBMt = 64 * WG_M, kAcc = BN_WG / 2;
   static_assert(EPI != EPI_LN || (WG_M == 1 && BN_WG == 232), "LN epilogue is laid out for 464 = 2 x 232 columns");
@@ -184,178 +181,305 @@
 
   const int warp = __shfl_sync(0xffffffffu, threadIdx.x >> 5, 0), lane = threadIdx.x & 31;
   const int num_kb = SM::R::num_kb(p.K);
-  const int n_mblk = p.M / kBMt, n_work = n_mblk * p.n_tiles;
-  const auto tile_m0 = [&](int t) { const int mb = t / p.n_tiles; return (p.rev ? n_mblk - 1 - mb : mb) * kBMt; };
-  const auto tile_n0 = [&](int t) { return (t % p.n_tiles) * BN_WG * SM::R::kWgN; };
+  const int n_mblk = p.M / kBMt;
+  const int mb = blockIdx.x / p.n_tiles;
+  const int m0 = (p.rev ? n_mblk - 1 - mb : mb) * kBMt, n0 = (blockIdx.x % p.n_tiles) * BN_WG * SM::R::kWgN;
 
   if (threadIdx.x == kGemmConsumers) {
     ring.prefetch(map_a, map_b);
-    if constexpr (STAGED) tma_prefetch_desc(&map_out);
     ring.init();
     fence_mbar_init();
   }
   __syncthreads();
   pdl_sync();
 
+  int s = 0;
+  uint32_t phase = 0;
   if (warp >= kGemmConsumers / 32) {
-    if constexpr (STAGED) setmaxnreg_dec<kProducerRegs>();
-    if (threadIdx.x == kGemmConsumers) {
-      int s = 0;
-      uint32_t phase = 0;
-      for (int t = blockIdx.x; t < n_work; t += gridDim.x) {
-        ring.load_tile(s, phase, map_a, map_b, num_kb, tile_m0(t), tile_n0(t));
-        if constexpr (!STAGED) break;
-      }
-    }
+    if (threadIdx.x == kGemmConsumers) ring.load_tile(s, phase, map_a, map_b, num_kb, m0, n0);
     return;
   }
 
-  if constexpr (STAGED) setmaxnreg_inc<kConsumerRegs>();
   const int wg = warp >> 2;
   const int wm = WG_M == 2 ? wg : 0, wn = WG_M == 2 ? 0 : wg;
   float acc[kAcc];
 #pragma unroll
   for (int i = 0; i < kAcc; ++i) acc[i] = 0.0f;
-  int s = 0;
-  uint32_t phase = 0;
-  for (int t = blockIdx.x; t < n_work; t += gridDim.x) {
-    const int m0 = tile_m0(t), n0 = tile_n0(t);
-    ring.template mma_tile<MODE>(s, phase, acc, wm, wn, num_kb, p.K);
-
-    const int rw = (warp & 3) * 16 + (lane >> 2);
-    const int row0 = m0 + wm * 64 + rw, row1 = row0 + 8;
-    const int col0 = n0 + wn * BN_WG + 2 * (lane & 3);
-
-    if constexpr (STAGED) {
+  ring.template mma_tile<MODE>(s, phase, acc, wm, wn, num_kb, p.K);
+
+  const int rw = (warp & 3) * 16 + (lane >> 2);
+  const int row0 = m0 + wm * 64 + rw, row1 = row0 + 8;
+  const int col0 = n0 + wn * BN_WG + 2 * (lane & 3);
+
+  if constexpr (EPI != EPI_LN) {
+    float scale = 1.0f;
+    if constexpr (EPI == EPI_QKV) scale = (n0 < p.qcols) ? p.qscale : 1.0f;
+#pragma unroll
+    for (int j = 0; j < BN_WG / 8; ++j) {
+      const int c = col0 + 8 * j;
+      if (c >= p.N) continue;
+      float v[4];
+      bias_act<EPI>(acc, j, p.bias, c, scale, v);
+      if constexpr (EPI == EPI_F32) {
+        float* o = static_cast<float*>(p.out);
+        *reinterpret_cast<float2*>(o + static_cast<size_t>(row0) * p.ldo + c) = make_float2(v[0], v[1]);
+        *reinterpret_cast<float2*>(o + static_cast<size_t>(row1) * p.ldo + c) = make_float2(v[2], v[3]);
+      } else {
+        uint32_t* o0 = reinterpret_cast<uint32_t*>(static_cast<typename O::T*>(p.out) + static_cast<size_t>(row0) * p.ldo + c);
+        uint32_t* o1 = reinterpret_cast<uint32_t*>(static_cast<typename O::T*>(p.out) + static_cast<size_t>(row1) * p.ldo + c);
+        if constexpr (SPLIT) {
+          uint32_t* l0 = reinterpret_cast<uint32_t*>(static_cast<typename O::T*>(p.out_lo) + static_cast<size_t>(row0) * p.ldo + c);
+          uint32_t* l1 = reinterpret_cast<uint32_t*>(static_cast<typename O::T*>(p.out_lo) + static_cast<size_t>(row1) * p.ldo + c);
+          O::pack_pair(v[0], v[1], *o0, *l0);
+          O::pack_pair(v[2], v[3], *o1, *l1);
+        } else {
+          *o0 = O::pack(v[0], v[1]);
+          *o1 = O::pack(v[2], v[3]);
+        }
+      }
+    }
+  } else {
+    float* ssum = reinterpret_cast<float*>(smem + SM::kOffStat);
+    float* ssq = ssum + 2 * 64;
+    const int N = p.N;
+    const float* r0p = p.resid + static_cast<size_t>(row0) * N;
+    const float* r1p = p.resid + static_cast<size_t>(row1) * N;
+    const float piv0 = __ldg(p.bias) + r0p[0], piv1 = __ldg(p.bias) + r1p[0];
+    float s0 = 0.0f, s1 = 0.0f;
+#pragma unroll
+    for (int j = 0; j < BN_WG / 8; ++j) {
+      const int c = col0 + 8 * j;
+      const float2 b = __ldg(reinterpret_cast<const float2*>(p.bias + c));
+      const float2 ra = *reinterpret_cast<const float2*>(r0p + c), rb = *reinterpret_cast<const float2*>(r1p + c);
+      acc[4 * j] += b.x + ra.x; acc[4 * j + 1] += b.y + ra.y;
+      acc[4 * j + 2] += b.x + rb.x; acc[4 * j + 3] += b.y + rb.y;
+      if (p.y_out != nullptr) {
+        *reinterpret_cast<float2*>(p.y_out + static_cast<size_t>(row0) * N + c) = make_float2(acc[4 * j], acc[4 * j + 1]);
+        *reinterpret_cast<float2*>(p.y_out + static_cast<size_t>(row1) * N + c) = make_float2(acc[4 * j + 2], acc[4 * j + 3]);
+      }
+      acc[4 * j] -= piv0; acc[4 * j + 1] -= piv0; acc[4 * j + 2] -= piv1; acc[4 * j + 3] -= piv1;
+      s0 += acc[4 * j] + acc[4 * j + 1];
+      s1 += acc[4 * j + 2] + acc[4 * j + 3];
+    }
+#pragma unroll
+    for (int o = 1; o <= 2; o <<= 1) {
+      s0 += __shfl_xor_sync(0xffffffffu, s0, o);
+      s1 += __shfl_xor_sync(0xffffffffu, s1, o);
+    }
+    if ((lane & 3) == 0) { ssum[wn * 64 + rw] = s0; ssum[wn * 64 + rw + 8] = s1; }
+    named_bar_sync(1, kGemmConsumers);
+    const float inv_n = 1.0f / static_cast<float>(N);
+    const float mean0 = (s0 + ssum[(wn ^ 1) * 64 + rw]) * inv_n, mean1 = (s1 + ssum[(wn ^ 1) * 64 + rw + 8]) * inv_n;
+    float q0 = 0.0f, q1 = 0.0f;
+#pragma unroll
+    for (int j = 0; j < BN_WG / 8; ++j) {
+      const float d0 = acc[4 * j] - mean0, d1 = acc[4 * j + 1] - mean0, d2 = acc[4 * j + 2] - mean1, d3 = acc[4 * j + 3] - mean1;
+      q0 = fmaf(d0, d0, fmaf(d1, d1, q0));
+      q1 = fmaf(d2, d2, fmaf(d3, d3, q1));
+    }
+#pragma unroll
+    for (int o = 1; o <= 2; o <<= 1) {
+      q0 += __shfl_xor_sync(0xffffffffu, q0, o);
+      q1 += __shfl_xor_sync(0xffffffffu, q1, o);
+    }
+    if ((lane & 3) == 0) { ssq[wn * 64 + rw] = q0; ssq[wn * 64 + rw + 8] = q1; }
+    named_bar_sync(1, kGemmConsumers);
+    const float rstd0 = 1.0f / sqrtf(fmaxf((q0 + ssq[(wn ^ 1) * 64 + rw]) * inv_n, 0.0f) + 1e-5f);
+    const float rstd1 = 1.0f / sqrtf(fmaxf((q1 + ssq[(wn ^ 1) * 64 + rw + 8]) * inv_n, 0.0f) + 1e-5f);
+    const LnAffine a = ln_affine(p.ln_scale, p.ln_shift, p.adaln, p.t_layout, p.n_layouts, m0, N);
+    typename O::T* out16 = static_cast<typename O::T*>(p.out);
+#pragma unroll
+    for (int j = 0; j < BN_WG / 8; ++j) {
+      const int c = col0 + 8 * j;
+      const float2 g = __ldg(reinterpret_cast<const float2*>(a.gam + c)), h = __ldg(reinterpret_cast<const float2*>(a.bet + c));
+      const float v0 = (acc[4 * j] - mean0) * rstd0 * (g.x + a.gadd) + h.x, v1 = (acc[4 * j + 1] - mean0) * rstd0 * (g.y + a.gadd) + h.y;
+      const float v2 = (acc[4 * j + 2] - mean1) * rstd1 * (g.x + a.gadd) + h.x, v3 = (acc[4 * j + 3] - mean1) * rstd1 * (g.y + a.gadd) + h.y;
+      if constexpr (SPLIT) {
+        typename O::T* lo16 = static_cast<typename O::T*>(p.out_lo);
+        O::pack_pair(v0, v1, *reinterpret_cast<uint32_t*>(out16 + static_cast<size_t>(row0) * N + c), *reinterpret_cast<uint32_t*>(lo16 + static_cast<size_t>(row0) * N + c));
+        O::pack_pair(v2, v3, *reinterpret_cast<uint32_t*>(out16 + static_cast<size_t>(row1) * N + c), *reinterpret_cast<uint32_t*>(lo16 + static_cast<size_t>(row1) * N + c));
+      } else {
+        *reinterpret_cast<uint32_t*>(out16 + static_cast<size_t>(row0) * N + c) = O::pack(v0, v1);
+        *reinterpret_cast<uint32_t*>(out16 + static_cast<size_t>(row1) * N + c) = O::pack(v2, v3);
+      }
+      if (p.out32 != nullptr) {
+        *reinterpret_cast<float2*>(p.out32 + static_cast<size_t>(row0) * N + c) = make_float2(v0, v1);
+        *reinterpret_cast<float2*>(p.out32 + static_cast<size_t>(row1) * N + c) = make_float2(v2, v3);
+      }
+    }
+  }
+}
+
+constexpr int kRbThreads = 384;
+struct RbSmem {
+  static constexpr int kKB = 64, kCols = 128, kAKb = 8;
+  using R = Ring<kKB, 1, 0, kCols, 1, 4, true, 128>;
+  static constexpr int kAKbBytes = kBM * 2 * kKB;
+  static constexpr int kOffRing = kAKb * kAKbBytes;
+  static constexpr int kStoreBytes = kBM * 128;
+  static constexpr int kOffStore = kOffRing + R::kBytes;
+  static constexpr int kOffBars = kOffStore + 2 * kStoreBytes;
+  static constexpr int kBytes = kOffBars + (2 * R::kStages + 2 * kAKb) * 8 + 1024 ;
+  static_assert(kBytes <= 232448, "exceeds the 227 KB of shared memory per CTA");
+};
+
+template <int EPI, int MODE>
+__global__ void __launch_bounds__(kRbThreads, 1)
+gemm_rowblock_kernel(const __grid_constant__ OpMaps<MODE> map_a , const __grid_constant__ OpMaps<MODE> map_b ,
+                     const __grid_constant__ CUtensorMap map_out , const GemmParams p) {
+  static_assert(EPI == EPI_QKV || EPI == EPI_RELU, "16-bit plain epilogues only");
+  static_assert(!kOpSplit<MODE>, "the split mode runs gemm_tc_kernel");
+  using SM = RbSmem;
+  using R = SM::R;
+  using O = OpT<MODE>;
+  constexpr int kKB = SM::kKB, kCols = SM::kCols;
+
+  extern __shared__ __align__(1024) uint8_t smem_raw[];
+  uint8_t* smem = reinterpret_cast<uint8_t*>((reinterpret_cast<uintptr_t>(smem_raw) + 1023) & ~uintptr_t(1023));
+  uint64_t* bars = reinterpret_cast<uint64_t*>(smem + SM::kOffBars);
+  R ring(smem + SM::kOffRing, bars);
+  uint64_t* a_full = bars + 2 * R::kStages;
+  uint64_t* a_empty = a_full + SM::kAKb;
+
+  const int warp = __shfl_sync(0xffffffffu, threadIdx.x >> 5, 0), lane = threadIdx.x & 31;
+  const int num_kb = R::num_kb(p.K);
+  const int n_mblk = p.M / kBM, n_items = n_mblk * p.n_ranges;
+  const auto item = [&](int w, int& m0, int& j0, int& j1) {
+    const int mb = w / p.n_ranges, r = w - mb * p.n_ranges;
+    m0 = (p.rev ? n_mblk - 1 - mb : mb) * kBM;
+    j0 = r * p.n_tiles / p.n_ranges; j1 = (r + 1) * p.n_tiles / p.n_ranges;
+  };
+
+  if (threadIdx.x == kGemmConsumers) {
+    R::prefetch(map_a, map_b);
+    tma_prefetch_desc(&map_out);
+    ring.init();
+    for (int kb = 0; kb < SM::kAKb; ++kb) { mbar_init(&a_full[kb], 1); mbar_init(&a_empty[kb], kGemmConsumers); }
+    fence_mbar_init();
+  }
+  __syncthreads();
+  pdl_sync();
+
+  if (warp >= kGemmConsumers / 32) {
+    setmaxnreg_dec<kProducerRegs>();
+    if (threadIdx.x == kGemmConsumers) {
+      int s = 0;
+      uint32_t phase = 0, ip = 0;
+      for (int w = blockIdx.x; w < n_items; w += gridDim.x, ip ^= 1) {
+        int m0, j0, j1;
+        item(w, m0, j0, j1);
+        for (int j = j0; j < j1; ++j) {
+          const auto load_a = [&](int kb) {
+            if (j != j0) return;
+            mbar_wait(&a_empty[kb], ip ^ 1);
+            mbar_arrive_expect_tx(&a_full[kb], SM::kAKbBytes);
+            tma_load_2d(smem + kb * SM::kAKbBytes, &map_a.hi, &a_full[kb], kb * kKB, m0);
+          };
+          ring.load_tile(s, phase, map_b, map_b, num_kb, 0, j * kCols, load_a);
+        }
+      }
+    }
+    return;
+  }
+
+  setmaxnreg_inc<kConsumerRegs>();
+  const int wg = warp >> 2;
+  const bool leader = (threadIdx.x & 127) == 0;
+  const auto wait_turn = [&]() { if (wg == 0) named_bar_sync(4, kGemmConsumers); else named_bar_sync(5, kGemmConsumers); };
+  const auto pass_turn = [&]() { if (wg == 0) named_bar_arrive(5, kGemmConsumers); else named_bar_arrive(4, kGemmConsumers); };
+  const auto wg_bar = [&]() { if (wg == 0) named_bar_sync(2, 128); else named_bar_sync(3, 128); };
+  int n_cta_tiles = 0;
+  for (int w = blockIdx.x; w < n_items; w += gridDim.x) { int m0, j0, j1; item(w, m0, j0, j1); n_cta_tiles += j1 - j0; }
+
+  float acc[2][kCols / 2];
+#pragma unroll
+  for (int h = 0; h < 2; ++h)
+#pragma unroll
+    for (int i = 0; i < kCols / 2; ++i) acc[h][i] = 0.0f;
+  const uint32_t a_base = smem_u32(smem);
+  uint8_t* stage = smem + SM::kOffStore + wg * SM::kStoreBytes;
+  const uint32_t stage_u32 = smem_u32(stage);
+  const int rw = (warp & 3) * 16 + (lane >> 2);
+  const int sw = (rw & 7) << 4;
+  int s = 0, q = 0;
+  uint32_t phase = 0, ip = 0;
+  for (int w = blockIdx.x; w < n_items; w += gridDim.x, ip ^= 1) {
+    int m0, j0, j1;
+    item(w, m0, j0, j1);
+    bool mine_any = false;
+    for (int j = j0; j < j1; ++j, ++q) {
+      if ((q & 1) != wg) {
+        for (int kb = 0; kb < num_kb; ++kb) R::advance(s, phase);
+        continue;
+      }
+      mine_any = true;
+      const bool last_mine = j + 2 >= j1;
+      const int n0 = j * kCols;
+      if (q > 0) wait_turn();
+      for (int kb = 0; kb < num_kb; ++kb) {
+        mbar_wait(&a_full[kb], ip);
+        mbar_wait(&ring.full[s], phase);
+        const uint64_t da = make_smem_desc<2 * kKB>(a_base + kb * SM::kAKbBytes);
+        const uint64_t db = make_smem_desc<2 * kKB>(smem_u32(ring.stages + s * R::kStageBytes));
+        wgmma_fence();
+        const auto step = [&](int k) {
+          wgmma_ss<kOpBf16<MODE>, kCols>(acc[0], da + 2 * k, db + 2 * k, (kb | k) != 0);
+          wgmma_ss<kOpBf16<MODE>, kCols>(acc[1], da + 512 + 2 * k, db + 2 * k, (kb | k) != 0);
+        };
+        const bool whole = kb * kKB + kKB <= p.K;
+        if (!whole) step(0);
+        if (whole) {
+#pragma unroll
+          for (int k = 0; k < kKB / kWgK; ++k) step(k);
+        }
+        wgmma_commit();
+        if (kb > 0) {
+          wgmma_wait<1>();
+          ring.release_prev(s);
+          if (last_mine) mbar_arrive(&a_empty[kb - 1]);
+        }
+        R::advance(s, phase);
+      }
+      if (q + 1 < n_cta_tiles) pass_turn();
+      wgmma_wait<0>();
+      fence_acc(acc[0]);
+      fence_acc(acc[1]);
+      ring.release_prev(s);
+      if (last_mine) mbar_arrive(&a_empty[num_kb - 1]);
+
       float scale = 1.0f;
       if constexpr (EPI == EPI_QKV) scale = (n0 < p.qcols) ? p.qscale : 1.0f;
-      const bool leader = (threadIdx.x & 127) == 0;
-      uint8_t* stage = smem + SM::kOffStore + wm * 64 * 128;
-      const uint32_t stage_u32 = smem_u32(stage);
-      const auto wg_bar = [&]() { if (wg == 0) named_bar_sync(2, 128); else named_bar_sync(3, 128); };
-      if (leader) bulk_wait_group_read<0>();
-      wg_bar();
-      const int sw = (rw & 7) << 4;
-#pragma unroll
-      for (int j = 0; j < BN_WG / 8; ++j) {
-        const int c = col0 + 8 * j;
-        if (c >= p.N) continue;
-        float v[4];
-        bias_act<EPI>(acc, j, p.bias, c, scale, v);
-        const uint32_t blk = stage_u32 + (j >> 3) * SM::kStoreCb + ((((j & 7) << 4) ^ sw) | (4 * (lane & 3)));
-        st_shared_u32(blk + rw * 128, O::pack(v[0], v[1]));
-        st_shared_u32(blk + (rw + 8) * 128, O::pack(v[2], v[3]));
-      }
-      fence_proxy_async_smem();
-      wg_bar();
-      if (leader) {
-#pragma unroll
-        for (int cb = 0; cb < BN_WG / 64; ++cb)
-          if (n0 + cb * 64 < p.N) tma_store_2d(&map_out, stage + cb * SM::kStoreCb, n0 + cb * 64, m0 + wm * 64);
-        bulk_commit_group();
-      }
-    } else if constexpr (EPI != EPI_LN) {
-      float scale = 1.0f;
-      if constexpr (EPI == EPI_QKV) scale = (n0 < p.qcols) ? p.qscale : 1.0f;
-#pragma unroll
-      for (int j = 0; j < BN_WG / 8; ++j) {
-        const int c = col0 + 8 * j;
-        if (c >= p.N) continue;
-        float v[4];
-        bias_act<EPI>(acc, j, p.bias, c, scale, v);
-        if constexpr (EPI == EPI_F32) {
-          float* o = static_cast<float*>(p.out);
-          *reinterpret_cast<float2*>(o + static_cast<size_t>(row0) * p.ldo + c) = make_float2(v[0], v[1]);
-          *reinterpret_cast<float2*>(o + static_cast<size_t>(row1) * p.ldo + c) = make_float2(v[2], v[3]);
-        } else {
-          uint32_t* o0 = reinterpret_cast<uint32_t*>(static_cast<typename O::T*>(p.out) + static_cast<size_t>(row0) * p.ldo + c);
-          uint32_t* o1 = reinterpret_cast<uint32_t*>(static_cast<typename O::T*>(p.out) + static_cast<size_t>(row1) * p.ldo + c);
-          if constexpr (SPLIT) {
-            uint32_t* l0 = reinterpret_cast<uint32_t*>(static_cast<typename O::T*>(p.out_lo) + static_cast<size_t>(row0) * p.ldo + c);
-            uint32_t* l1 = reinterpret_cast<uint32_t*>(static_cast<typename O::T*>(p.out_lo) + static_cast<size_t>(row1) * p.ldo + c);
-            O::pack_pair(v[0], v[1], *o0, *l0);
-            O::pack_pair(v[2], v[3], *o1, *l1);
-          } else {
-            *o0 = O::pack(v[0], v[1]);
-            *o1 = O::pack(v[2], v[3]);
+      const int col0 = n0 + 2 * (lane & 3);
+#pragma unroll
+      for (int cb = 0; cb < kCols / 64; ++cb) {
+        if (n0 + cb * 64 >= p.N) continue;
+        if (leader) bulk_wait_group_read<0>();
+        wg_bar();
+#pragma unroll
+        for (int j8 = 8 * cb; j8 < 8 * cb + 8; ++j8) {
+          const int c = col0 + 8 * j8;
+          const uint32_t blk = stage_u32 + ((((j8 & 7) << 4) ^ sw) | (4 * (lane & 3)));
+#pragma unroll
+          for (int h = 0; h < 2; ++h) {
+            float v[4];
+            bias_act<EPI>(acc[h], j8, p.bias, c, scale, v);
+            st_shared_u32(blk + (h * 64 + rw) * 128, O::pack(v[0], v[1]));
+            st_shared_u32(blk + (h * 64 + rw + 8) * 128, O::pack(v[2], v[3]));
           }
         }
-      }
-    } else {
-      float* ssum = reinterpret_cast<float*>(smem + SM::kOffStat);
-      float* ssq = ssum + 2 * 64;
-      const int N = p.N;
-      const float* r0p = p.resid + static_cast<size_t>(row0) * N;
-      const float* r1p = p.resid + static_cast<size_t>(row1) * N;
-      const float piv0 = __ldg(p.bias) + r0p[0], piv1 = __ldg(p.bias) + r1p[0];
-      float s0 = 0.0f, s1 = 0.0f;
-#pragma unroll
-      for (int j = 0; j < BN_WG / 8; ++j) {
-        const int c = col0 + 8 * j;
-        const float2 b = __ldg(reinterpret_cast<const float2*>(p.bias + c));
-        const float2 ra = *reinterpret_cast<const float2*>(r0p + c), rb = *reinterpret_cast<const float2*>(r1p + c);
-        acc[4 * j] += b.x + ra.x; acc[4 * j + 1] += b.y + ra.y;
-        acc[4 * j + 2] += b.x + rb.x; acc[4 * j + 3] += b.y + rb.y;
-        if (p.y_out != nullptr) {
-          *reinterpret_cast<float2*>(p.y_out + static_cast<size_t>(row0) * N + c) = make_float2(acc[4 * j], acc[4 * j + 1]);
-          *reinterpret_cast<float2*>(p.y_out + static_cast<size_t>(row1) * N + c) = make_float2(acc[4 * j + 2], acc[4 * j + 3]);
-        }
-        acc[4 * j] -= piv0; acc[4 * j + 1] -= piv0; acc[4 * j + 2] -= piv1; acc[4 * j + 3] -= piv1;
-        s0 += acc[4 * j] + acc[4 * j + 1];
-        s1 += acc[4 * j + 2] + acc[4 * j + 3];
-      }
-#pragma unroll
-      for (int o = 1; o <= 2; o <<= 1) {
-        s0 += __shfl_xor_sync(0xffffffffu, s0, o);
-        s1 += __shfl_xor_sync(0xffffffffu, s1, o);
-      }
-      if ((lane & 3) == 0) { ssum[wn * 64 + rw] = s0; ssum[wn * 64 + rw + 8] = s1; }
-      named_bar_sync(1, kGemmConsumers);
-      const float inv_n = 1.0f / static_cast<float>(N);
-      const float mean0 = (s0 + ssum[(wn ^ 1) * 64 + rw]) * inv_n, mean1 = (s1 + ssum[(wn ^ 1) * 64 + rw + 8]) * inv_n;
-      float q0 = 0.0f, q1 = 0.0f;
-#pragma unroll
-      for (int j = 0; j < BN_WG / 8; ++j) {
-        const float d0 = acc[4 * j] - mean0, d1 = acc[4 * j + 1] - mean0, d2 = acc[4 * j + 2] - mean1, d3 = acc[4 * j + 3] - mean1;
-        q0 = fmaf(d0, d0, fmaf(d1, d1, q0));
-        q1 = fmaf(d2, d2, fmaf(d3, d3, q1));
-      }
-#pragma unroll
-      for (int o = 1; o <= 2; o <<= 1) {
-        q0 += __shfl_xor_sync(0xffffffffu, q0, o);
-        q1 += __shfl_xor_sync(0xffffffffu, q1, o);
-      }
-      if ((lane & 3) == 0) { ssq[wn * 64 + rw] = q0; ssq[wn * 64 + rw + 8] = q1; }
-      named_bar_sync(1, kGemmConsumers);
-      const float rstd0 = 1.0f / sqrtf(fmaxf((q0 + ssq[(wn ^ 1) * 64 + rw]) * inv_n, 0.0f) + 1e-5f);
-      const float rstd1 = 1.0f / sqrtf(fmaxf((q1 + ssq[(wn ^ 1) * 64 + rw + 8]) * inv_n, 0.0f) + 1e-5f);
-      const LnAffine a = ln_affine(p.ln_scale, p.ln_shift, p.adaln, p.t_layout, p.n_layouts, m0, N);
-      typename O::T* out16 = static_cast<typename O::T*>(p.out);
-#pragma unroll
-      for (int j = 0; j < BN_WG / 8; ++j) {
-        const int c = col0 + 8 * j;
-        const float2 g = __ldg(reinterpret_cast<const float2*>(a.gam + c)), h = __ldg(reinterpret_cast<const float2*>(a.bet + c));
-        const float v0 = (acc[4 * j] - mean0) * rstd0 * (g.x + a.gadd) + h.x, v1 = (acc[4 * j + 1] - mean0) * rstd0 * (g.y + a.gadd) + h.y;
-        const float v2 = (acc[4 * j + 2] - mean1) * rstd1 * (g.x + a.gadd) + h.x, v3 = (acc[4 * j + 3] - mean1) * rstd1 * (g.y + a.gadd) + h.y;
-        if constexpr (SPLIT) {
-          typename O::T* lo16 = static_cast<typename O::T*>(p.out_lo);
-          O::pack_pair(v0, v1, *reinterpret_cast<uint32_t*>(out16 + static_cast<size_t>(row0) * N + c), *reinterpret_cast<uint32_t*>(lo16 + static_cast<size_t>(row0) * N + c));
-          O::pack_pair(v2, v3, *reinterpret_cast<uint32_t*>(out16 + static_cast<size_t>(row1) * N + c), *reinterpret_cast<uint32_t*>(lo16 + static_cast<size_t>(row1) * N + c));
-        } else {
-          *reinterpret_cast<uint32_t*>(out16 + static_cast<size_t>(row0) * N + c) = O::pack(v0, v1);
-          *reinterpret_cast<uint32_t*>(out16 + static_cast<size_t>(row1) * N + c) = O::pack(v2, v3);
-        }
-        if (p.out32 != nullptr) {
-          *reinterpret_cast<float2*>(p.out32 + static_cast<size_t>(row0) * N + c) = make_float2(v0, v1);
-          *reinterpret_cast<float2*>(p.out32 + static_cast<size_t>(row1) * N + c) = make_float2(v2, v3);
-        }
-      }
-    }
-    if constexpr (!STAGED) break;
-  }
-  if constexpr (STAGED) {
-    if ((threadIdx.x & 127) == 0) bulk_wait_group_all();
-  }
+        fence_proxy_async_smem();
+        wg_bar();
+        if (leader) {
+          tma_store_2d(&map_out, stage, n0 + cb * 64, m0);
+          bulk_commit_group();
+        }
+      }
+    }
+    if (!mine_any) {
+      for (int kb = 0; kb < num_kb; ++kb) { mbar_wait(&a_full[kb], ip); mbar_arrive(&a_empty[kb]); }
+    }
+  }
+  if (leader) bulk_wait_group_all();
 }
 
 constexpr int kLnThreads = 384, kLnEpiThreads = 96;
diff --git a/layoutdm_b200/csrc/ldm_b200.cu b/layoutdm_b200/csrc/ldm_b200.cu
--- a/layoutdm_b200/csrc/ldm_b200.cu
+++ b/layoutdm_b200/csrc/ldm_b200.cu
@@ -40,25 +40,22 @@
 constexpr int kMaxLayouts = 32767;
 constexpr int kLogitLd = 160;
 constexpr int kDModel = 464;
-constexpr int kPlainBN = 256;
-template <int MODE> constexpr int kPlainStages = kOpSplit<MODE> ? 4 : 3;
+constexpr int kPlainBN = 256, kPlainStages = 4;
+constexpr int kRbCols = RbSmem::kCols;
+static_assert(kDModel <= RbSmem::kAKb * RbSmem::kKB && kAttN % kRbCols == 0 && kQkvN % 64 == 0 && 4 * kDModel % 64 == 0,
+              "row-block GEMM shapes: K fits the resident A, Q tiles are whole tiles, N is whole 64-column store blocks");
 constexpr int kHeadBN = 160, kHeadStages = 4;
 constexpr int kLnBN = 232, kLnStages = 3;
 constexpr int kLnKB = LnSmem::R::kKB;
 static_assert(LnSmem::kWgCols == kLnBN && kAttN % kLnKB == 0 && 4 * kDModel % kLnKB == 0 && gemm_kb(true) == kLnKB, "LN GEMM shapes");
-template <int MODE> constexpr auto kGemmQkv = gemm_tc_kernel<kPlainBN, 2, kPlainStages<MODE>, EPI_QKV, MODE>;
-template <int MODE> constexpr auto kGemmFf1 = gemm_tc_kernel<kPlainBN, 2, kPlainStages<MODE>, EPI_RELU, MODE>;
+template <int EPI, int MODE> constexpr auto kGemmPlainSplit = gemm_tc_kernel<kPlainBN, 2, kPlainStages, EPI, MODE>;
 template <int MODE> constexpr auto kGemmHead = gemm_tc_kernel<kHeadBN, 2, kHeadStages, EPI_F32, MODE>;
 template <int MODE> constexpr auto kGemmLn = gemm_tc_kernel<kLnBN, 1, kLnStages, EPI_LN, MODE>;
-template <int MODE>
-constexpr int kPlainSmem = GemmSmem<kPlainBN, 2, kPlainStages<MODE>, kOpSplit<MODE>, kStagedStore<EPI_QKV, kOpSplit<MODE>>>::kBytes;
+constexpr int kPlainSmem = GemmSmem<kPlainBN, 2, kPlainStages, true>::kBytes;
 constexpr int kHeadSmem = GemmSmem<kHeadBN, 2, kHeadStages>::kBytes;
 constexpr int kLnSmem = GemmSmem<kLnBN, 1, kLnStages>::kBytes;
-static_assert(GemmSmem<kHeadBN, 2, kHeadStages, true>::kBytes == kHeadSmem && GemmSmem<kLnBN, 1, kLnStages, true>::kBytes == kLnSmem &&
-              GemmSmem<kPlainBN, 2, 4, true>::R::kStageBytes == GemmSmem<kPlainBN, 2, 4>::R::kStageBytes,
+static_assert(GemmSmem<kHeadBN, 2, kHeadStages, true>::kBytes == kHeadSmem && GemmSmem<kLnBN, 1, kLnStages, true>::kBytes == kLnSmem,
               "split-mode ring stages must keep the one-plane sizes");
-static_assert(kStagedStore<EPI_QKV, false> == kStagedStore<EPI_RELU, false> && kStagedStore<EPI_QKV, true> == kStagedStore<EPI_RELU, true>,
-              "QKV and FF1 share one shared-memory size");
 
 using EncodeTiledFn = CUresult (*)(CUtensorMap*, CUtensorMapDataType, cuuint32_t, void*, const cuuint64_t*, const cuuint64_t*,
                                    const cuuint32_t*, const cuuint32_t*, CUtensorMapInterleave, CUtensorMapSwizzle,
@@ -146,6 +143,7 @@
   int num_sms = 0;
   int max_threads_sm = 0;
   int gemm_ctas = 0;
+  int gemm_split = 0;
   int fuse_embed = 1;
   cudaStream_t cap_stream = nullptr;
   cudaGraphExec_t graph_exec = nullptr;
@@ -317,8 +315,13 @@
 template <int MODE>
 int set_smem() {
   constexpr auto attr = cudaFuncAttributeMaxDynamicSharedMemorySize;
-  CK(cudaFuncSetAttribute(kGemmQkv<MODE>, attr, kPlainSmem<MODE>));
-  CK(cudaFuncSetAttribute(kGemmFf1<MODE>, attr, kPlainSmem<MODE>));
+  if constexpr (kOpSplit<MODE>) {
+    CK(cudaFuncSetAttribute(kGemmPlainSplit<EPI_QKV, MODE>, attr, kPlainSmem));
+    CK(cudaFuncSetAttribute(kGemmPlainSplit<EPI_RELU, MODE>, attr, kPlainSmem));
+  } else {
+    CK(cudaFuncSetAttribute(gemm_rowblock_kernel<EPI_QKV, MODE>, attr, RbSmem::kBytes));
+    CK(cudaFuncSetAttribute(gemm_rowblock_kernel<EPI_RELU, MODE>, attr, RbSmem::kBytes));
+  }
   CK(cudaFuncSetAttribute(kGemmHead<MODE>, attr, kHeadSmem));
   if constexpr (kOpSplit<MODE>) CK(cudaFuncSetAttribute(kGemmLn<MODE>, attr, kLnSmem));
   else CK(cudaFuncSetAttribute(gemm_ln_kernel<MODE>, attr, LnSmem::kBytes));
@@ -378,14 +381,15 @@
   h->cap = n_layouts;
   h->ws_generation++;
   int rc;
+  static_assert(gemm_kb(false) == RbSmem::kKB, "one A geometry for QKV / FF1 / head");
   const int kb = gemm_kb(h->split);
   if ((rc = make_op_maps(h, &h->m_x16, &h->m_x16_lo, h->x16, h->x16_lo, M, d, kBM, kb))) return rc;
   if ((rc = make_op_maps(h, &h->m_z16, &h->m_z16_lo, h->z16, h->z16_lo, M, d, kBM, kb))) return rc;
   if ((rc = make_op_maps(h, &h->m_att16, &h->m_att16_lo, h->att16, h->att16_lo, M, kAttN, 64, kLnKB))) return rc;
   if ((rc = make_op_maps(h, &h->m_hid16, &h->m_hid16_lo, h->hid16, h->hid16_lo, M, ff, 64, kLnKB))) return rc;
   if ((rc = make_op_maps(h, &h->m_qkv16, &h->m_qkv16_lo, h->qkv16, h->qkv16_lo, M, kQkvN, kBM, kHeadPad))) return rc;
-  if (!h->split && (rc = make_map(&h->m_qkv16_st, h->qkv16, M, kQkvN, 64, 64, h->bf16))) return rc;
-  if (!h->split && (rc = make_map(&h->m_hid16_st, h->hid16, M, ff, 64, 64, h->bf16))) return rc;
+  if (!h->split && (rc = make_map(&h->m_qkv16_st, h->qkv16, M, kQkvN, kBM, 64, h->bf16))) return rc;
+  if (!h->split && (rc = make_map(&h->m_hid16_st, h->hid16, M, ff, kBM, 64, h->bf16))) return rc;
   return LDM_OK;
 }
 
@@ -398,10 +402,20 @@
     if (!persistent) return dim3(tiles);
     return dim3(std::min({tiles, h->num_sms, h->gemm_ctas > 0 ? h->gemm_ctas : tiles}));
   };
-  const CUtensorMap no_store{};
-  constexpr bool kStaged = kStagedStore<EPI_QKV, kOpSplit<MODE>>;
+  const auto plain_gemm = [&](auto epi, const OpMaps<MODE>& a, const OpMaps<MODE>& w, const CUtensorMap& out, GemmParams p) {
+    constexpr int EPI = decltype(epi)::value;
+    if constexpr (kOpSplit<MODE>) {
+      p.n_tiles = (p.N + kPlainBN - 1) / kPlainBN;
+      return launch_step(h, kGemmPlainSplit<EPI, MODE>, grid(p.n_tiles * n, false), kGemmThreads, kPlainSmem, st, a, w, p);
+    } else {
+      p.n_tiles = (p.N + kRbCols - 1) / kRbCols;
+      const int g = h->gemm_split > 0 ? h->gemm_split : n >= h->num_sms ? 1 : (h->num_sms + n - 1) / n;
+      p.n_ranges = std::min(g, p.n_tiles);
+      return launch_step(h, gemm_rowblock_kernel<EPI, MODE>, grid(n * p.n_ranges, true), kRbThreads, RbSmem::kBytes, st, a, w, out, p);
+    }
+  };
   const auto ln_gemm = [&](const OpMaps<MODE>& a, const OpMaps<MODE>& w, const GemmParams& p) {
-    if constexpr (kOpSplit<MODE>) return launch_step(h, kGemmLn<MODE>, grid(M / 64, false), kGemmThreads<EPI_LN, MODE>, kLnSmem, st, a, w, no_store, p);
+    if constexpr (kOpSplit<MODE>) return launch_step(h, kGemmLn<MODE>, grid(M / 64, false), kGemmThreads, kLnSmem, st, a, w, p);
     else return launch_step(h, gemm_ln_kernel<MODE>, grid(M / 64, true), kLnThreads, LnSmem::kBytes, st, a, w, p);
   };
   int done = 0;
@@ -417,11 +431,10 @@
   if (!skip_embed) LDM_STAGE_DONE();
   for (int l = 0; l < L; ++l) {
     {
-      GemmParams p{M, kQkvN, d, kQkvN / kPlainBN, h->bqkv[l], h->qkv16, kQkvN, 1.0f / sqrtf(static_cast<float>(d / h->desc.n_heads)), 8 * kHeadPad};
+      GemmParams p{M, kQkvN, d, 0, h->bqkv[l], h->qkv16, kQkvN, 1.0f / sqrtf(static_cast<float>(d / h->desc.n_heads)), 8 * kHeadPad};
       p.rev = next_rev(); p.out_lo = h->qkv16_lo;
       ProfScope ps(h, CAT_QKV, st);
-      CK(launch_step(h, kGemmQkv<MODE>, grid(p.n_tiles * n, kStaged), kGemmThreads<EPI_QKV, MODE>, kPlainSmem<MODE>, st, maps(h->m_x16, h->m_x16_lo), maps(h->m_wqkv[l], h->m_wqkv_lo[l]),
-                     kStaged ? h->m_qkv16_st : no_store, p));
+      CK(plain_gemm(std::integral_constant<int, EPI_QKV>{}, maps(h->m_x16, h->m_x16_lo), maps(h->m_wqkv[l], h->m_wqkv_lo[l]), h->m_qkv16_st, p));
     }
     LDM_STAGE_DONE();
     {
@@ -438,11 +451,10 @@
     }
     LDM_STAGE_DONE();
     {
-      GemmParams p{M, ff, d, (ff + kPlainBN - 1) / kPlainBN, h->b1[l], h->hid16, ff, 1.0f, 0};
+      GemmParams p{M, ff, d, 0, h->b1[l], h->hid16, ff, 1.0f, 0};
       p.rev = next_rev(); p.out_lo = h->hid16_lo;
       ProfScope ps(h, CAT_FF1, st);
-      CK(launch_step(h, kGemmFf1<MODE>, grid(p.n_tiles * n, kStaged), kGemmThreads<EPI_RELU, MODE>, kPlainSmem<MODE>, st, maps(h->m_z16, h->m_z16_lo), maps(h->m_w1[l], h->m_w1_lo[l]),
-                     kStaged ? h->m_hid16_st : no_store, p));
+      CK(plain_gemm(std::integral_constant<int, EPI_RELU>{}, maps(h->m_z16, h->m_z16_lo), maps(h->m_w1[l], h->m_w1_lo[l]), h->m_hid16_st, p));
     }
     LDM_STAGE_DONE();
     {
@@ -464,7 +476,7 @@
     GemmParams p{M, kLogitLd, d, 1, nullptr, h->logits, kLogitLd, 1.0f, 0};
     p.rev = next_rev();
     ProfScope ps(h, CAT_HEAD, st);
-    CK(launch_step(h, kGemmHead<MODE>, grid(n, false), kGemmThreads<EPI_F32, MODE>, kHeadSmem, st, maps(h->m_z16, h->m_z16_lo), maps(h->m_whead, h->m_whead_lo), no_store, p));
+    CK(launch_step(h, kGemmHead<MODE>, grid(n, false), kGemmThreads, kHeadSmem, st, maps(h->m_z16, h->m_z16_lo), maps(h->m_whead, h->m_whead_lo), p));
   }
 #undef LDM_STAGE_DONE
   CK(cudaGetLastError());
@@ -652,6 +664,7 @@
   h->num_sms = prop.multiProcessorCount;
   h->max_threads_sm = prop.maxThreadsPerMultiProcessor;
   if (const char* e = getenv("LDM_GEMM_CTAS")) h->gemm_ctas = std::max(1, atoi(e));
+  if (const char* e = getenv("LDM_GEMM_SPLIT")) h->gemm_split = std::max(1, atoi(e));
 #define TRY(x) do { rc = (x); if (rc) { ldm_destroy(h); return rc; } } while (0)
 
   TRY(dev_alloc(h, &h->cat_emb, static_cast<size_t>(C) * d));
@@ -659,6 +672,7 @@
   TRY(dev_alloc(h, &h->hlnw, static_cast<size_t>(d)));
   TRY(dev_alloc(h, &h->hlnb, static_cast<size_t>(d)));
   TRY(dev_alloc(h, &h->adaln, static_cast<size_t>(L) * T * 2 * d));
+  const int plain_w_rows = h->split ? kPlainBN : kRbCols;
   for (int l = 0; l < L; ++l) {
     TRY(alloc16(h, &h->wqkv[l], &h->wqkv_lo[l], kQkvN, d));
     TRY(alloc16(h, &h->wo[l], &h->wo_lo[l], d, kAttN));
@@ -670,9 +684,9 @@
     TRY(dev_alloc(h, &h->b2[l], static_cast<size_t>(d)));
     TRY(dev_alloc(h, &h->ln2w[l], static_cast<size_t>(d)));
     TRY(dev_alloc(h, &h->ln2b[l], static_cast<size_t>(d)));
-    TRY(make_op_maps(h, &h->m_wqkv[l], &h->m_wqkv_lo[l], h->wqkv[l], h->wqkv_lo[l], kQkvN, d, kPlainBN, gemm_kb(h->split)));
+    TRY(make_op_maps(h, &h->m_wqkv[l], &h->m_wqkv_lo[l], h->wqkv[l], h->wqkv_lo[l], kQkvN, d, plain_w_rows, gemm_kb(h->split)));
     TRY(make_op_maps(h, &h->m_wo[l], &h->m_wo_lo[l], h->wo[l], h->wo_lo[l], d, kAttN, kLnBN, kLnKB));
-    TRY(make_op_maps(h, &h->m_w1[l], &h->m_w1_lo[l], h->w1[l], h->w1_lo[l], ff, d, kPlainBN, gemm_kb(h->split)));
+    TRY(make_op_maps(h, &h->m_w1[l], &h->m_w1_lo[l], h->w1[l], h->w1_lo[l], ff, d, plain_w_rows, gemm_kb(h->split)));
     TRY(make_op_maps(h, &h->m_w2[l], &h->m_w2_lo[l], h->w2[l], h->w2_lo[l], d, ff, kLnBN, kLnKB));
   }
   TRY(alloc16(h, &h->whead, &h->whead_lo, kLogitLd, d));
```

New measurement: 1047 (median of 6 runs). 1.06x the previous value.
